# wengroup/matten

Measured on AMD Instinct MI355X. Metric: edge_tensor_products_per_sec, higher is better.
Workload: dtype f32; 1 GPU; configs[2]: synthetic fcc-64 crystals (64 atoms, cutoff 5 A, 1152 edges each), paper hparams lmax=4, eval forward backbone+out_layer, one batch per step per GPU; last conv layer run for its live outputs only (258/842 radial-weight columns: the irreps its only reader takes) -- `value` counts 4 edge-TP per edge all the same, `value_full_layers` is the rate with the full last layer; nodes_per_gpu=64000, edges_per_gpu=1152000, conv_layers=4

## Files before the change

### include/matten_hip.h

```cpp
#ifndef MATTEN_HIP_H
#define MATTEN_HIP_H

#include <stddef.h>
#include <stdint.h>

#ifdef __cplusplus
extern "C" {
#endif

typedef void* matten_stream_t;

#define MATTEN_OK 0
#define MATTEN_EINVAL (-1)
#define MATTEN_ELAUNCH (-2)
#define MATTEN_ENOMEM (-3)

int matten_abi_version(void);

#define MATTEN_RADIAL_MAX_MID 3

size_t matten_csr_workspace_bytes(int64_t n_edges, int64_t n_nodes);
int matten_csr_counting_max_avg_degree(void);
int matten_csr_build(const int64_t* edge_index, int64_t n_edges, int64_t n_nodes, int32_t* perm,
                     int32_t* rowptr, int32_t* src_sorted, void* workspace, size_t workspace_bytes,
                     int32_t* err_flag, matten_stream_t stream);

int64_t matten_csr_split_bound(int64_t n_nodes, int64_t n_edges, int64_t max_len);
int matten_csr_split(const int32_t* rowptr, int64_t n_nodes, int64_t n_edges, int64_t max_len, int32_t* vrowptr,
                     int64_t* vseg, const float* num_neigh, float* vnn, matten_stream_t stream);

size_t matten_group_workspace_bytes(int64_t n, int64_t n_keys);
int matten_group_by_key(const int64_t* key, int64_t n, int64_t n_keys, int32_t* order, int32_t* seg,
                        void* workspace, size_t workspace_bytes, int32_t* err_flag, matten_stream_t stream);

int matten_species_embed(const int64_t* atomic_numbers, int64_t n_nodes, const int64_t* z_to_index,
                         int64_t min_z, int64_t max_z, int64_t n_species, const float* weight ,
                         const float* bias , int64_t dim, int64_t* species_index, int32_t* species_i32,
                         float* node_feats, float* node_attrs, int32_t* err_flag, matten_stream_t stream);

int matten_edge_geom(const float* pos, const int64_t* edge_index, const float* edge_cell_shift,
                     const float* cell, int64_t n_cells, const int64_t* batch, const int32_t* perm,
                     int64_t n_edges, int64_t n_nodes, int lmax, int n_basis, float r_start, float r_end,
                     float* geom_sorted, float* sh_sorted, int sh_stride, float* edge_vectors, float* edge_lengths,
                     float* edge_attrs, float* edge_embedding, matten_stream_t stream);

int matten_radial_mlp(const float* geom_sorted, int64_t n_edges, int n_basis, float r_start, float r_end,
                      const float* w0p, int nb_pad, const float* w1p, const float* w2p, int hidden, int w_pad,
                      float act_cst, void* w_edge, int out_is_bf16, matten_stream_t stream);
int matten_radial_mlp_deep(const float* geom_sorted, int64_t n_edges, int n_basis, float r_start, float r_end,
                           const float* w0p, int nb_pad, const float* w_mid, int n_mid, const float* w2p, int hidden,
                           int w_pad, float act_cst, void* w_edge, int out_is_bf16, matten_stream_t stream);

int matten_tp_tile_nodes(void);
int matten_tp_paths(const float* x, int64_t d_in, const void* w_edge, int64_t w_pad, const float* sh_sorted,
                    int64_t sh_dim, const int32_t* rowptr, const int32_t* src_sorted, int64_t n_nodes,
                    const int32_t* path_entries, const int32_t* unit_start, int64_t n_entries,
                    int64_t units_per_tile, int64_t d_mid, float avg_num_neighbors, const float* num_neigh,
                    float* agg , int w_is_bf16, matten_stream_t stream);

int matten_agg_linear_max_mt(void);
int matten_agg_linear_block_chunks(void);
size_t matten_agg_linear_lds_bytes(int64_t w_stride, int64_t n_io, int64_t n_blocks);
size_t matten_agg_linear_max_lds_bytes(void);
int matten_agg_linear(const float* agg, int64_t ld, const int32_t* order, const int32_t* seg, int64_t n_species,
                      const float* wtab, int64_t w_stride, const int32_t* io_table, int64_t n_io,
                      const int32_t* blocks, int64_t n_blocks, const float* add, int64_t add_ld, int64_t d_out,
                      int64_t n_rows, float* out, matten_stream_t stream);
int matten_agg_linear_gate(const float* agg, int64_t ld, const int32_t* order, const int32_t* seg, int64_t n_species,
                           const float* wtab, int64_t w_stride, const int32_t* io_table, int64_t n_io,
                           const int32_t* blocks, int64_t n_blocks, const float* add, int64_t add_ld, int64_t d_out,
                           int64_t n_rows, const int32_t* cmeta, const float* act_cst, const float* bn_scale,
                           const float* bn_shift, int64_t d_act, float* out, matten_stream_t stream);
int matten_agg_linear_gate_sets(void);
int matten_radial_hidden(const float* geom_sorted, int64_t n_edges, int n_basis, float r_start, float r_end,
                         const float* w0p, int nb_pad, const float* w1p, int hidden, uint16_t* h2s,
                         const float* h_scale, matten_stream_t stream);
int matten_radial_hidden_multi(const float* geom_sorted, int64_t n_edges, int n_basis, float r_start, float r_end,
                               const float* const* w0p, int nb_pad, const float* const* w1p, int hidden,
                               uint16_t* const* h2s, const float* const* h_scale, int n_layers,
                               matten_stream_t stream);
int matten_radial_hidden_deep(const float* geom_sorted, int64_t n_edges, int n_basis, float r_start, float r_end,
                              const float* w0p, int nb_pad, const float* w_mid, int n_mid, int hidden, uint16_t* h2s,
                              const float* h_scale, matten_stream_t stream);
int matten_radial_hidden_multi_deep(const float* geom_sorted, int64_t n_edges, int n_basis, float r_start, float r_end,
                                    const float* const* w0p, int nb_pad, const float* const* w_mid, int n_mid, int hidden,
                                    uint16_t* const* h2s, const float* const* h_scale, int n_layers,
                                    matten_stream_t stream);
int matten_tp_fused(const float* x, int64_t d_in, const uint16_t* h2s, const float* w2p, int64_t w_pad,
                    const float* sh_sorted, int64_t sh_stride, const int32_t* rowptr, const int32_t* src_sorted,
                    int64_t n_nodes, const int32_t* group_entries, const int32_t* unit_map, int64_t n_entries,
                    int64_t units_per_tile, int64_t lds_floats_per_wave, int64_t d_mid, float avg_num_neighbors,
                    const float* num_neigh, const uint16_t* a_split, const float* a_scale_inv,
                    float* agg , matten_stream_t stream);

int matten_tp_max_cols(void);
int matten_tp_max_cols_l0(void);
int matten_tp_max_cols_l1(void);
int matten_tp_groups_hash(void);

int matten_species_linear(const float* x, int64_t d_in, const int32_t* order, const int32_t* seg, int64_t n_species,
                          const float* wp, int64_t w_stride, const int32_t* segs, int64_t n_segs, int64_t d_out,
                          const float* add, int64_t add_ld, int64_t n_rows, float* out, matten_stream_t stream);

int matten_species_linear_rows(const float* x, int64_t d_in, const int32_t* order, const int32_t* seg, int64_t n_species,
                               const float* wp, int64_t w_stride, const int32_t* segs, int64_t n_segs, int64_t d_out,
                               const float* add, int64_t add_ld, int64_t n_rows, float* out, matten_stream_t stream);

int matten_gate_bn(const float* x, int64_t d_in, const int32_t* meta, int64_t d_out, const float* act_cst,
                   const float* running_mean, const float* running_var, const float* bn_weight,
                   const float* bn_bias, float eps, int64_t n_rows, float* out, matten_stream_t stream);

int matten_segment_reduce(const float* x, int64_t dim, const int64_t* ptr, int64_t n_segments, int mean,
                          float* out, matten_stream_t stream);
int matten_segment_minmax(const float* x, int64_t dim, const int64_t* ptr, int64_t n_segments, int take_max, float* out,
                          int64_t* arg, matten_stream_t stream);
int matten_segment_minmax_bwd(const float* dy, int64_t dim, const int64_t* arg, int64_t n_segments, float* dx,
                              matten_stream_t stream);

int64_t matten_radial_mlp_bwd_small_slices(int64_t n_edges);
int64_t matten_radial_mlp_bwd_w2_ranges(int64_t n_edges, int64_t w_pad);
int matten_radial_mlp_bwd(const float* geom_sorted, int64_t n_edges, int n_basis, float r_start, float r_end,
                          const float* w0p, int nb_pad, const float* w1p, const float* w2p, int hidden, int w_pad,
                          int w_cols, const void* dw, int64_t dw_ld, int dw_is_bf16, float* h2_scratch,
                          float* part_small, float* part_w2, float scale0, float scale1, float scale2,
                          float* grad_small, float* grad_w2, matten_stream_t stream);
int64_t matten_radial_mlp_bwd_w2_ranges_deep(int64_t n_edges, int64_t w_pad, int n_mid);
int matten_radial_mlp_bwd_deep(const float* geom_sorted, int64_t n_edges, int n_basis, float r_start, float r_end,
                               const float* w0p, int nb_pad, const float* w_mid, int n_mid, const float* w2p, int hidden,
                               int w_pad, int w_cols, const void* dw, int64_t dw_ld, int dw_is_bf16, float* h2_scratch,
                               float* part_small, float* part_w2, float scale0, float scale1, float scale2,
                               float* grad_small, float* grad_w2, matten_stream_t stream);
int matten_radial_pack(const float* w0, const float* w1, const float* w2, int n_basis, int nb_pad, int w_cols, int w_pad,
                       float scale0, float scale1, float scale2, float* w0p, float* w1p, float* w2p,
                       matten_stream_t stream);
int matten_radial_pack_deep(const float* w0, const float* w_mid, int n_mid, const float* w2, int n_basis, int nb_pad,
                            int w_cols, int w_pad, float scale0, float scale1, float scale2, float* w0p, float* w_mid_p,
                            float* w2p, matten_stream_t stream);
int matten_radial_pack_cols(const float* w0, const float* w1, const float* w2, int n_basis, int nb_pad, int w_cols,
                            const int64_t* cols, int n_cols, int w_pad, float scale0, float scale1, float scale2, float* w0p,
                            float* w1p, float* w2p, matten_stream_t stream);
int matten_radial_h_scale(const float* w0, const float* w1, int n_basis, float r_start, float r_end, float act_cst,
                          float* out2, matten_stream_t stream);
int matten_radial_pack_cols_deep(const float* w0, const float* w_mid, int n_mid, const float* w2, int n_basis, int nb_pad,
                                 int w_cols, const int64_t* cols, int n_cols, int w_pad, float scale0, float scale1,
                                 float scale2, float* w0p, float* w_mid_p, float* w2p, matten_stream_t stream);
int matten_radial_h_scale_deep(const float* w0, const float* w_mid, int n_mid, int n_basis, float r_start, float r_end,
                               float act_cst, float* out2, matten_stream_t stream);
int matten_split_a_tiles(const float* w2p, int64_t w_pad, const int32_t* group_entries, int64_t n_entries,
                         const float* h_scale, uint16_t* frag, float* scale_inv, matten_stream_t stream);
int matten_gather_scale(const float* src, const int64_t* idx, const float* scale, int64_t n, int64_t scale_period,
                        int scale_by_source, float* out, const int64_t* perm2, float* out2, matten_stream_t stream);
int64_t matten_species_linear_wgrad_scratch_floats(int64_t n_rows, int64_t n_species, int64_t w_stride);

int matten_dense_rows(const float* x, int64_t n_in, const float* q, int64_t n_out, int64_t n_rows, float* out,
                      matten_stream_t stream);



int matten_tp_backward(const float* x, int64_t d_in, const void* w_edge, int64_t w_ld, const float* sh_sorted,
                       int64_t sh_stride, const int32_t* src_sorted, const int32_t* dst_sorted,
                       const int32_t* col_meta, int64_t n_cols, const uint8_t* nnz_ijk, const float* nnz_c,
                       const float* g_agg, int64_t d_mid, float avg_num_neighbors, const float* num_neigh,
                       int64_t n_edges, float* dx, void* dw, int64_t dw_ld, const int32_t* in_ptr,
                       const int32_t* in_cols, int64_t n_in, int edge_is_bf16 ,
                       matten_stream_t stream);

int matten_adam_step(float* params, const float* grads, float* exp_avg, float* exp_avg_sq, int64_t n, const float* step,
                     float lr, float beta1, float beta2, float eps, float weight_decay, matten_stream_t stream);

int matten_tp_backward_lit(const float* x, int64_t d_in, const void* w_edge, int64_t w_ld, const float* sh_sorted,
                           int64_t sh_stride, const int32_t* src_sorted, const int32_t* dst_sorted, const int32_t* blocks,
                           int64_t n_blocks, int64_t max_mul, const int32_t* paths, int64_t n_paths, const float* g_agg,
                           int64_t d_mid, float avg_num_neighbors, const float* num_neigh, int64_t n_edges, float* dx,
                           void* dw, int64_t dw_ld, int edge_is_bf16, int64_t n_nodes, const int32_t* out_ptr,
                           const int32_t* out_perm, float* dx_edges, int max_l, matten_stream_t stream);
int matten_tp_backward_lit_wfree(const float* x, int64_t d_in, const uint16_t* h2s, const uint16_t* frag, const float* w_inv,
                                 const float* sh_sorted, int64_t sh_stride, const int32_t* src_sorted,
                                 const int32_t* dst_sorted, const int32_t* blocks, int64_t n_blocks, int64_t sum_lanes,
                                 const int32_t* paths, int64_t n_paths, const float* g_agg, int64_t d_mid,
                                 float avg_num_neighbors, const float* num_neigh, int64_t n_edges, float* dx, void* dw,
                                 int64_t dw_ld, int edge_is_bf16, int64_t n_nodes, const int32_t* out_ptr,
                                 const int32_t* out_perm, float* dx_edges, int64_t lds_floats, int max_l, int max_mul,
                                 matten_stream_t stream);

int matten_species_linear_wgrad(const float* x, int64_t d_in, const float* dy, int64_t d_out, const int32_t* order,
                                const int32_t* seg, int64_t n_species, int64_t n_rows, const int32_t* segs,
                                int64_t n_segs, int64_t w_stride, float* dwp, float* scratch, matten_stream_t stream);

int matten_gate_bwd(const float* x, int64_t d_in, const int32_t* meta, int64_t d_out, const float* act_cst,
                    const float* dy, int64_t n_rows, float* dx, matten_stream_t stream);

int64_t matten_bn_scratch_floats(int64_t n_rows, int64_t dim);
int matten_bn_train_fwd(const float* x, int64_t dim, int64_t n_rows, const int32_t* col2chan, const int32_t* chan,
                        int64_t n_chan, const float* weight, const float* bias, float eps, float* mean, float* nu,
                        float* y, float* running_mean, float* running_var, float momentum, float* scratch,
                        matten_stream_t stream);
int matten_bn_train_bwd(const float* x, const float* dy, int64_t dim, int64_t n_rows, const int32_t* col2chan,
                        const int32_t* chan, int64_t n_chan, const float* mean, const float* nu, const float* weight,
                        float eps, float* A, float* B, float* dx, float* dweight, float* dbias, float* scratch,
                        matten_stream_t stream);

int matten_norm_act(const float* x, int64_t dim, int64_t n_rows, const int32_t* chan, int64_t n_chan, int act,
                    float epsilon, const float* running_mean, const float* running_var, const float* bn_weight,
                    const float* bn_bias, float bn_eps, float* y, matten_stream_t stream);
int matten_norm_act_bwd(const float* x, const float* dy, int64_t dim, int64_t n_rows, const int32_t* chan, int64_t n_chan,
                        int act, float epsilon, float* dx, matten_stream_t stream);

int matten_instance_norm_fwd(const float* x, int64_t dim, int64_t n_rows, const int64_t* seg_ptr, const int64_t* seg_of_row,
                             int64_t n_seg, const int32_t* col2chan, const int32_t* chan, int64_t n_chan,
                             const float* weight, const float* bias, float eps, float* mean, float* nu, float* y,
                             matten_stream_t stream);
int matten_instance_norm_bwd(const float* x, const float* dy, int64_t dim, int64_t n_rows, const int64_t* seg_ptr,
                             const int64_t* seg_of_row, int64_t n_seg, const int32_t* col2chan, const int32_t* chan,
                             int64_t n_chan, const float* mean, const float* nu, const float* weight, float eps, float* A,
                             float* B, float* dx, matten_stream_t stream);

int matten_segment_reduce_bwd(const float* dy, int64_t dim, const int64_t* ptr, int64_t n_segments, int mean, float* dx,
                              matten_stream_t stream);


int matten_graph_prep(const double* pos, const double* cell, const int64_t* ptr, int64_t n_crystals, double r_cut,
                      double* frac, double* bound, int64_t* batch, float* pos_f32, float* cell_f32,
                      matten_stream_t stream);
int matten_neighbor_count(const double* pos, const double* cell, const int64_t* ptr, const double* frac,
                          const double* bound, const int64_t* pair_ptr, double r_cut, int64_t n_crystals,
                          int64_t max_atoms, int32_t* counts, int32_t* counts_t, matten_stream_t stream);
int matten_neighbor_summary(const int64_t* offsets, const int64_t* pair_ptr, int64_t n_crystals, int64_t* out2,
                            matten_stream_t stream);
int matten_neighbor_fill(const double* pos, const double* cell, const int64_t* ptr, const double* frac,
                         const double* bound, const int64_t* pair_ptr, double r_cut, int64_t n_crystals,
                         int64_t max_atoms, const int64_t* offsets, int64_t n_edges, int64_t* edge_index,
                         float* edge_cell_shift, float* num_neigh, const int64_t* offsets_t, int64_t n_atoms,
                         int32_t* rowptr, int32_t* src_sorted, int32_t* perm, matten_stream_t stream);

#ifdef __cplusplus
}
#endif
#endif
```

### matten_amd/_lib.py

```python
from __future__ import annotations

import ctypes
import os
from ctypes import c_float, c_int, c_int32, c_int64, c_size_t, c_void_p

_HERE = os.path.dirname(os.path.abspath(__file__))
LIB_PATH = os.path.join(_HERE, "libmatten_hip.so")

ABI_VERSION = 45

P = c_void_p
SIGNATURES = {
    "matten_abi_version": (c_int, []),
    "matten_csr_workspace_bytes": (c_size_t, [c_int64, c_int64]),
    "matten_group_workspace_bytes": (c_size_t, [c_int64, c_int64]),
    "matten_csr_counting_max_avg_degree": (c_int, []),
    "matten_csr_build": (c_int, [P, c_int64, c_int64, P, P, P, P, c_size_t, P, P]),
    "matten_csr_split_bound": (c_int64, [c_int64, c_int64, c_int64]),
    "matten_csr_split": (c_int, [P, c_int64, c_int64, c_int64, P, P, P, P, P]),
    "matten_group_by_key": (c_int, [P, c_int64, c_int64, P, P, P, c_size_t, P, P]),
    "matten_species_embed": (c_int, [P, c_int64, P, c_int64, c_int64, c_int64, P, P, c_int64, P, P, P, P, P, P]),
    "matten_edge_geom": (c_int, [P, P, P, P, c_int64, P, P, c_int64, c_int64, c_int, c_int, c_float, c_float, P, P, c_int, P, P, P, P, P]),
    "matten_radial_mlp": (c_int, [P, c_int64, c_int, c_float, c_float, P, c_int, P, P, c_int, c_int, c_float, P, c_int, P]),
    "matten_radial_mlp_deep": (c_int, [P, c_int64, c_int, c_float, c_float, P, c_int, P, c_int, P, c_int, c_int, c_float, P, c_int,
                                       P]),
    "matten_tp_tile_nodes": (c_int, []),
    "matten_tp_paths": (c_int, [P, c_int64, P, c_int64, P, c_int64, P, P, c_int64, P, P, c_int64, c_int64, c_int64, c_float, P, P, c_int,
                                P]),
    "matten_radial_hidden_multi": (c_int, [P, c_int64, c_int, c_float, c_float, P, c_int, P, c_int, P, P, c_int, P]),
    "matten_radial_hidden_multi_deep": (c_int, [P, c_int64, c_int, c_float, c_float, P, c_int, P, c_int, c_int, P, P, c_int, P]),
    "matten_agg_linear_max_mt": (c_int, []),
    "matten_agg_linear_block_chunks": (c_int, []),
    "matten_agg_linear_lds_bytes": (c_size_t, [c_int64, c_int64, c_int64]),
    "matten_agg_linear_max_lds_bytes": (c_size_t, []),
    "matten_agg_linear": (c_int, [P, c_int64, P, P, c_int64, P, c_int64, P, c_int64, P, c_int64, P, c_int64, c_int64,
                                  c_int64, P, P]),
    "matten_agg_linear_gate": (c_int, [P, c_int64, P, P, c_int64, P, c_int64, P, c_int64, P, c_int64, P, c_int64, c_int64,
                                       c_int64, P, P, P, P, c_int64, P, P]),
    "matten_agg_linear_gate_sets": (c_int, []),
    "matten_radial_hidden": (c_int, [P, c_int64, c_int, c_float, c_float, P, c_int, P, c_int, P, P, P]),
    "matten_radial_hidden_deep": (c_int, [P, c_int64, c_int, c_float, c_float, P, c_int, P, c_int, c_int, P, P, P]),
    "matten_tp_max_cols": (c_int, []),
    "matten_tp_max_cols_l0": (c_int, []),
    "matten_tp_max_cols_l1": (c_int, []),
    "matten_tp_groups_hash": (c_int, []),
    "matten_tp_fused": (c_int, [P, c_int64, P, P, c_int64, P, c_int64, P, P, c_int64, P, P, c_int64, c_int64, c_int64, c_int64, c_float, P, P, P, P, P]),
    "matten_species_linear": (c_int, [P, c_int64, P, P, c_int64, P, c_int64, P, c_int64, c_int64, P, c_int64, c_int64, P, P]),
    "matten_species_linear_rows": (c_int, [P, c_int64, P, P, c_int64, P, c_int64, P, c_int64, c_int64, P, c_int64, c_int64, P, P]),
    "matten_radial_mlp_bwd_small_slices": (c_int64, [c_int64]),
    "matten_radial_mlp_bwd_w2_ranges": (c_int64, [c_int64, c_int64]),
    "matten_radial_mlp_bwd_w2_ranges_deep": (c_int64, [c_int64, c_int64, c_int]),
    "matten_radial_mlp_bwd": (c_int, [P, c_int64, c_int, c_float, c_float, P, c_int, P, P, c_int, c_int, c_int, P, c_int64,
                                      c_int, P, P, P, c_float, c_float, c_float, P, P, P]),
    "matten_radial_mlp_bwd_deep": (c_int, [P, c_int64, c_int, c_float, c_float, P, c_int, P, c_int, P, c_int, c_int, c_int, P,
                                           c_int64, c_int, P, P, P, c_float, c_float, c_float, P, P, P]),
    "matten_radial_pack": (c_int, [P, P, P, c_int, c_int, c_int, c_int, c_float, c_float, c_float, P, P, P, P]),
    "matten_radial_pack_deep": (c_int, [P, P, c_int, P, c_int, c_int, c_int, c_int, c_float, c_float, c_float, P, P, P, P]),
    "matten_radial_pack_cols": (c_int, [P, P, P, c_int, c_int, c_int, P, c_int, c_int, c_float, c_float, c_float, P, P, P, P]),
    "matten_radial_pack_cols_deep": (c_int, [P, P, c_int, P, c_int, c_int, c_int, P, c_int, c_int, c_float, c_float, c_float, P, P,
                                             P, P]),
    "matten_radial_h_scale": (c_int, [P, P, c_int, c_float, c_float, c_float, P, P]),
    "matten_radial_h_scale_deep": (c_int, [P, P, c_int, c_int, c_float, c_float, c_float, P, P]),
    "matten_split_a_tiles": (c_int, [P, c_int64, P, c_int64, P, P, P, P]),
    "matten_gather_scale": (c_int, [P, P, P, c_int64, c_int64, c_int, P, P, P, P]),
    "matten_species_linear_wgrad_scratch_floats": (c_int64, [c_int64, c_int64, c_int64]),
    "matten_tp_backward": (c_int, [P, c_int64, P, c_int64, P, c_int64, P, P, P, c_int64, P, P, P, c_int64, c_float, P, c_int64, P, P, c_int64,
                                   P, P, c_int64, c_int, P]),
    "matten_tp_backward_lit": (c_int, [P, c_int64, P, c_int64, P, c_int64, P, P, P, c_int64, c_int64, P, c_int64, P, c_int64, c_float,
                                       P, c_int64, P, P, c_int64, c_int, c_int64, P, P, P, c_int, P]),
    "matten_tp_backward_lit_wfree": (c_int, [P, c_int64, P, P, P, P, c_int64, P, P, P, c_int64, c_int64, P, c_int64, P, c_int64, c_float,
                                             P, c_int64, P, P, c_int64, c_int, c_int64, P, P, P, c_int64, c_int, c_int, P]),
    "matten_adam_step": (c_int, [P, P, P, P, c_int64, P, c_float, c_float, c_float, c_float, c_float, P]),
    "matten_species_linear_wgrad": (c_int, [P, c_int64, P, c_int64, P, P, c_int64, c_int64, P, c_int64, c_int64, P, P, P]),
    "matten_gate_bwd": (c_int, [P, c_int64, P, c_int64, P, P, c_int64, P, P]),
    "matten_bn_scratch_floats": (c_int64, [c_int64, c_int64]),
    "matten_bn_train_fwd": (c_int, [P, c_int64, c_int64, P, P, c_int64, P, P, c_float, P, P, P, P, P, c_float, P, P]),
    "matten_bn_train_bwd": (c_int, [P, P, c_int64, c_int64, P, P, c_int64, P, P, P, c_float, P, P, P, P, P, P, P]),
    "matten_norm_act": (c_int, [P, c_int64, c_int64, P, c_int64, c_int, c_float, P, P, P, P, c_float, P, P]),
    "matten_norm_act_bwd": (c_int, [P, P, c_int64, c_int64, P, c_int64, c_int, c_float, P, P]),
    "matten_instance_norm_fwd": (c_int, [P, c_int64, c_int64, P, P, c_int64, P, P, c_int64, P, P, c_float, P, P, P, P]),
    "matten_instance_norm_bwd": (c_int, [P, P, c_int64, c_int64, P, P, c_int64, P, P, c_int64, P, P, P, c_float, P, P, P, P]),
    "matten_segment_reduce_bwd": (c_int, [P, c_int64, P, c_int64, c_int, P, P]),
    "matten_graph_prep": (c_int, [P, P, P, c_int64, ctypes.c_double, P, P, P, P, P, P]),
    "matten_neighbor_count": (c_int, [P, P, P, P, P, P, ctypes.c_double, c_int64, c_int64, P, P, P]),
    "matten_neighbor_summary": (c_int, [P, P, c_int64, P, P]),
    "matten_neighbor_fill": (c_int, [P, P, P, P, P, P, ctypes.c_double, c_int64, c_int64, P, c_int64, P, P, P, P, c_int64,
                                     P, P, P, P]),
    "matten_gate_bn": (c_int, [P, c_int64, P, c_int64, P, P, P, P, P, c_float, c_int64, P, P]),
    "matten_segment_reduce": (c_int, [P, c_int64, P, c_int64, c_int, P, P]),
    "matten_segment_minmax": (c_int, [P, c_int64, P, c_int64, c_int, P, P, P]),
    "matten_segment_minmax_bwd": (c_int, [P, c_int64, P, c_int64, P, P]),
    "matten_dense_rows": (c_int, [P, c_int64, P, c_int64, c_int64, P, P]),
}

_lib = None


class MattenHipError(RuntimeError):
    pass


def load() -> ctypes.CDLL:
    global _lib
    if _lib is not None:
        return _lib
    if not os.path.exists(LIB_PATH):
        raise MattenHipError(
            f"{LIB_PATH} not found: the HIP extension is not built. matten_amd has no CPU fallback; "
            "run `make -C matten_amd/csrc` (needs hipcc, --offload-arch=gfx950)."
        )
    lib = ctypes.CDLL(LIB_PATH)
    for name, (res, args) in SIGNATURES.items():
        try:
            fn = getattr(lib, name)
        except AttributeError as e:
            raise MattenHipError(f"symbol {name} missing from {LIB_PATH}") from e
        fn.restype = res
        fn.argtypes = args
    v = lib.matten_abi_version()
    if v != ABI_VERSION:
        raise MattenHipError(f"ABI version mismatch: library {v}, python binding {ABI_VERSION}")
    _lib = lib
    return lib


_ERRORS = {-1: "MATTEN_EINVAL (bad argument)", -2: "MATTEN_ELAUNCH (HIP launch failed)", -3: "MATTEN_ENOMEM (workspace too small)"}


def check(rc: int, what: str) -> None:
    if rc != 0:
        raise MattenHipError(f"{what} failed: {_ERRORS.get(rc, rc)}")
```

### matten_amd/csrc/agg_linear.hip

```cpp
#include <atomic>

#include "common.h"

namespace {

typedef float f32x4 __attribute__((ext_vector_type(4)));

#ifndef AL_WAVES_PER_WG
#define AL_WAVES_PER_WG 8
#endif
constexpr int AL_WAVES = AL_WAVES_PER_WG;
constexpr int AL_ROWS = 16;
#ifndef AL_BLK_CHUNKS
#define AL_BLK_CHUNKS 4
#endif
#ifndef AL_MIN_BLOCKS
#define AL_MIN_BLOCKS 3
#endif
#ifndef AL_GATE_PREFETCH
#define AL_GATE_PREFETCH 1
#endif
constexpr int AL_BLK = AL_BLK_CHUNKS;
constexpr int AL_MAX_MT = 2;

constexpr int AL_STAGE_RS = 33;

struct AggIo {
    int chunk0, T, K, packed, a_off, out_off, mo, k0;
};
struct AggBlk {
    int chunk;
    int info;
    int t0;
    int pad;
};

struct Args {
    const float* agg;
    const int* order;
    const int* seg;
    const float* wtab;
    const AggIo* io;
    const AggBlk* blk;
    const float* add;
    float* out;
    int64_t ld;
    int n_species, w_stride, n_io, n_blk, add_ld, d_out, n_rows;
    const int4* cmeta;
    const float* act_cst;
    const float* bn_scale;
    const float* bn_shift;
    int out_ld;
};

__device__ __forceinline__ float al_act(int code, float v) {
    switch (code) {
        case 1: return v / (1.0f + expf(-v));
        case 2: return tanhf(v);
        case 3: return 1.0f / (1.0f + expf(-v));
        case 4: return (v > 20.0f ? v : log1pf(expf(v))) - 0.6931471805599453f;
        case 5: return fabsf(v);
        default: return v;
    }
}
constexpr int AL_GATE_SETS = 3;

#ifdef AL_WAVES_PER_EU
#define AL_OCC __attribute__((amdgpu_waves_per_eu(AL_WAVES_PER_EU, AL_WAVES_PER_EU)))
#else
#define AL_OCC
#endif
template <bool GATE>
__global__ __launch_bounds__(AL_WAVES * 64, AL_MIN_BLOCKS) AL_OCC void agg_linear_kernel(Args a) {
    extern __shared__ __attribute__((aligned(16))) float lds[];
    AggIo* io_l = reinterpret_cast<AggIo*>(lds + a.w_stride);
    AggBlk* blk_l = reinterpret_cast<AggBlk*>(io_l + a.n_io);
    float* stage_all = reinterpret_cast<float*>(blk_l + a.n_blk);
    int s = 0, blk = blockIdx.x, beg = 0, end = a.n_rows;
    if (a.order) {
        int* sseg = reinterpret_cast<int*>(stage_all);
        const int cap = AL_WAVES * (16 * AL_STAGE_RS + 16) - 4;
        if (a.n_species + 1 <= cap) {
            for (int i = threadIdx.x; i <= a.n_species; i += AL_WAVES * 64) sseg[i] = a.seg[i];
            __syncthreads();
            if (threadIdx.x == 0) {
                int b = blk, sp = 0;
                for (; sp < a.n_species; ++sp) {
                    const int nb = (sseg[sp + 1] - sseg[sp] + AL_WAVES * AL_ROWS - 1) / (AL_WAVES * AL_ROWS);
                    if (b < nb) break;
                    b -= nb;
                }
                sseg[cap] = sp;
                sseg[cap + 1] = b;
            }
            __syncthreads();
            s = sseg[cap];
            blk = sseg[cap + 1];
            if (s < a.n_species) beg = sseg[s], end = sseg[s + 1];
            __syncthreads();
        } else {
            for (; s < a.n_species; ++s) {
                beg = a.seg[s];
                end = a.seg[s + 1];
                const int nb = (end - beg + AL_WAVES * AL_ROWS - 1) / (AL_WAVES * AL_ROWS);
                if (blk < nb) break;
                blk -= nb;
            }
        }
    } else if (blk >= (a.n_rows + AL_WAVES * AL_ROWS - 1) / (AL_WAVES * AL_ROWS)) {
        s = a.n_species;
    }
    if (s >= a.n_species) return;
    {
        const f32x4* src = reinterpret_cast<const f32x4*>(a.wtab + (int64_t)s * a.w_stride);
        f32x4* dst = reinterpret_cast<f32x4*>(lds);
        for (int i = threadIdx.x; i < a.w_stride / 4; i += AL_WAVES * 64) dst[i] = src[i];
        const int* isrc = reinterpret_cast<const int*>(a.io);
        int* idst = reinterpret_cast<int*>(io_l);
        for (int i = threadIdx.x; i < a.n_io * 8; i += AL_WAVES * 64) idst[i] = isrc[i];
        const int* bsrc = reinterpret_cast<const int*>(a.blk);
        int* bdst = reinterpret_cast<int*>(blk_l);
        for (int i = threadIdx.x; i < a.n_blk * 4; i += AL_WAVES * 64) bdst[i] = bsrc[i];
    }
    __syncthreads();
    const int wave = __builtin_amdgcn_readfirstlane(threadIdx.x >> 6);
    const int lane = threadIdx.x & 63;
    const int g = lane >> 4, c = lane & 15;
    const int r0 = beg + (blk * AL_WAVES + wave) * AL_ROWS;
    if (r0 >= end) return;
    const int ri = min(r0 + c, end - 1);
    const bool row_ok = r0 + c < end;
    const int64_t row = a.order ? a.order[ri] : ri;
    const float* rp = a.agg + row * a.ld + 4 * g;
    const bool has_add = a.add != nullptr;
    float* stage = stage_all + wave * (16 * AL_STAGE_RS);
    int* rowid = reinterpret_cast<int*>(stage_all + AL_WAVES * 16 * AL_STAGE_RS) + wave * 16;
    if (g == 0) rowid[c] = row_ok ? (int)row : -1;
    const int fcol = lane & 31, frow = lane >> 5;

    int K = 0, d3 = 0, n_mt = 0, cw = 0, a_off = 0, out_off = 0, mo = 0, k0 = 0, kk = 1;
    auto load_io = [&](int ii) {
        const AggIo r = io_l[ii];
        K = __builtin_amdgcn_readfirstlane(r.K);
        d3 = __builtin_amdgcn_readfirstlane(r.packed & 255);
        n_mt = __builtin_amdgcn_readfirstlane((r.packed >> 8) & 255);
        cw = __builtin_amdgcn_readfirstlane((r.packed >> 16) & 255);
        a_off = __builtin_amdgcn_readfirstlane(r.a_off);
        out_off = __builtin_amdgcn_readfirstlane(r.out_off);
        mo = __builtin_amdgcn_readfirstlane(r.mo);
        k0 = __builtin_amdgcn_readfirstlane(r.k0);
        kk = __builtin_amdgcn_readfirstlane((r.packed >> 24) & 255);
    };
    f32x4 acc[AL_MAX_MT];
    float addv[8];
    auto zero_acc = [&]() {
#pragma unroll
        for (int mt = 0; mt < AL_MAX_MT; ++mt) acc[mt] = f32x4{0.f, 0.f, 0.f, 0.f};
    };
    int4 cm_row = {0, 0, 0, 0};
    float cst_row = 1.0f, bsc_row = 1.0f, bsh_row = 0.0f;
    int ocol = 0;
    auto open_row = [&]() {
        const int w = mo * kk;
        const int fc = min(fcol, w - 1), fv = fc / kk;
        ocol = out_off + fv * d3 + k0 + (fc - fv * kk);
#pragma unroll
        for (int p = 0; p < 8; ++p) {
            const int rid = max(rowid[2 * p + frow], 0);
            addv[p] = has_add ? a.add[(int64_t)rid * a.add_ld + ocol] : 0.0f;
        }
        if constexpr (GATE && AL_GATE_PREFETCH) {
            cm_row = a.cmeta[ocol];
            const int type = cm_row.x & 255, code = (cm_row.x >> 8) & 255;
            cst_row = code ? a.act_cst[code] : 1.0f;
            bsc_row = 1.0f, bsh_row = 0.0f;
            if (a.bn_scale && (type == 1 || type == 3)) bsc_row = a.bn_scale[cm_row.y], bsh_row = a.bn_shift[cm_row.y];
        }
    };
    auto close_unit = [&](int k) {
#pragma unroll
        for (int mt = 0; mt < AL_MAX_MT; ++mt) {
            if (mt < n_mt) {
#pragma unroll
                for (int i = 0; i < 4; ++i) {
                    const int v = 16 * mt + 4 * g + i;
                    if (v < mo) stage[c * AL_STAGE_RS + v * kk + (k - k0)] = acc[mt][i];
                }
            }
        }
    };
    float gate_reg[GATE ? AL_GATE_SETS : 1][8];
    auto flush_row = [&]() {
        const int w = mo * kk;
        __builtin_amdgcn_s_waitcnt(0xc07f);
        __builtin_amdgcn_wave_barrier();
        if constexpr (GATE) {
            const int4 cm = AL_GATE_PREFETCH ? cm_row : a.cmeta[ocol];
            const int type = cm.x & 255, code = (cm.x >> 8) & 255;
            float cst = cst_row, bsc = bsc_row, bsh = bsh_row;
            if (!AL_GATE_PREFETCH) {
                cst = code ? a.act_cst[code] : 1.0f;
                if (a.bn_scale && (type == 1 || type == 3)) bsc = a.bn_scale[cm.y], bsh = a.bn_shift[cm.y];
            }
            const int src_lane = (cm.z & 31) | (frow << 5);
#pragma unroll
            for (int p = 0; p < 8; ++p) {
                const int r = 2 * p + frow;
                const int rid = rowid[r];
                float v = stage[r * AL_STAGE_RS + min(fcol, w - 1)] + addv[p];
                float gv = __shfl(gate_reg[0][p], src_lane);
#pragma unroll
                for (int st = 1; st < AL_GATE_SETS; ++st) {
                    const float o = __shfl(gate_reg[st][p], src_lane);
                    gv = cm.w == st ? o : gv;
                }
                if (type == 2) {
                    const float act = (code ? al_act(code, v) : v) * cst;
#pragma unroll
                    for (int st = 0; st < AL_GATE_SETS; ++st)
                        if (cm.w == st && fcol < w) gate_reg[st][p] = act;
                } else if (fcol < w && rid >= 0 && type != 0) {
                    if (type == 1) v = (code ? al_act(code, v) : v) * cst;
                    else v = v * gv;
                    a.out[(int64_t)rid * a.out_ld + cm.y] = fmaf(v, bsc, bsh);
                }
            }
            __builtin_amdgcn_wave_barrier();
            return;
        }
#pragma unroll
        for (int p = 0; p < 8; ++p) {
            const int r = 2 * p + frow;
            const int rid = rowid[r];
#ifdef AL_ABL_NO_STORE
            if (fcol < w && rid >= 0 && addv[p] == 12345.678f)
#elif defined(AL_ABL_SMALL_OUT)
            if (fcol < w && rid >= 0) a.out[(int64_t)(rid & 63) * a.d_out + ocol] = stage[r * AL_STAGE_RS + fcol] + addv[p];
            if (false)
#else
            if (fcol < w && rid >= 0)
#endif
                a.out[(int64_t)rid * a.d_out + ocol] = stage[r * AL_STAGE_RS + fcol] + addv[p];
        }
        __builtin_amdgcn_wave_barrier();
    };
    auto fetch = [&](int j, f32x4* __restrict__ buf) {
        const AggBlk d = blk_l[j];
        const int c0 = __builtin_amdgcn_readfirstlane(d.chunk);
        const int n = __builtin_amdgcn_readfirstlane(d.info & 255);
#pragma unroll
        for (int i = 0; i < AL_BLK; ++i) {
#ifdef AL_NT_LOADS
            buf[i] = __builtin_nontemporal_load(reinterpret_cast<const f32x4*>(rp + 16 * (c0 + min(i, n - 1))));
#else
            buf[i] = *reinterpret_cast<const f32x4*>(rp + 16 * (c0 + min(i, n - 1)));
#endif
        }
    };
    auto step = [&](int j, const f32x4* __restrict__ cur, f32x4* __restrict__ nxt) {
        fetch(min(j + 1, a.n_blk - 1), nxt);
        const AggBlk d = blk_l[j];
        const int info = __builtin_amdgcn_readfirstlane(d.info);
        const int n = info & 255, k = (info >> 12) & 255;
        const int t0 = __builtin_amdgcn_readfirstlane(d.t0);
        const int cc = min(c, cw - 1);
#pragma unroll
        for (int i = 0; i < AL_BLK; ++i) {
            if (i < n) {
                f32x4 b = cur[i];
#ifdef AL_ABL_NO_LDS
                const f32x4 afix = {1.f, 2.f, 3.f, (float)i};
#endif
                const int t = t0 + i;
                const int slot0 = 16 * t + 4 * g;
#pragma unroll
                for (int sst = 0; sst < 4; ++sst) b[sst] = slot0 + sst < K ? b[sst] : 0.0f;
                const float* ab = lds + a_off + ((t * n_mt * 4 + g) * cw + cc) * 4;
#pragma unroll
                for (int mt = 0; mt < AL_MAX_MT; ++mt) {
                    if (mt < n_mt) {
#ifdef AL_ABL_NO_LDS
                        f32x4 a4 = afix;
#else
                        f32x4 a4 = *reinterpret_cast<const f32x4*>(ab + mt * 4 * cw * 4);
#endif
                        if (c >= cw) a4 = f32x4{0.f, 0.f, 0.f, 0.f};
#ifdef AL_ABL_NO_MFMA
                        acc[mt][0] += a4[0] * b[0] + a4[1] * b[1] + a4[2] * b[2] + a4[3] * b[3];
#else
#pragma unroll
                        for (int sst = 0; sst < 4; ++sst)
                            acc[mt] = __builtin_amdgcn_mfma_f32_16x16x4f32(a4[sst], b[sst], acc[mt], 0, 0, 0);
#endif
                    }
                }
            }
        }
        if ((info >> 9) & 1) {
            close_unit(k);
            zero_acc();
            if ((info >> 10) & 1) {
                flush_row();
                if (j + 1 < a.n_blk) {
                    load_io((__builtin_amdgcn_readfirstlane(blk_l[j + 1].info) >> 20) & 4095);
                    open_row();
                }
            }
        }
    };
#pragma unroll
    for (int st = 0; st < (GATE ? AL_GATE_SETS : 1); ++st)
#pragma unroll
        for (int p = 0; p < 8; ++p) gate_reg[st][p] = 0.0f;
    f32x4 bufa[AL_BLK], bufb[AL_BLK];
    __builtin_amdgcn_s_waitcnt(0xc07f);
    __builtin_amdgcn_wave_barrier();
    load_io(0);
    zero_acc();
    open_row();
    fetch(0, bufa);
    for (int j = 0; j < a.n_blk; j += 2) {
        step(j, bufa, bufb);
        if (j + 1 < a.n_blk) step(j + 1, bufb, bufa);
    }
}

}

constexpr size_t AL_MAX_LDS = 80 * 1024;
extern "C" size_t matten_agg_linear_lds_bytes(int64_t w_stride, int64_t n_io, int64_t n_blocks) {
    return sizeof(float) * (size_t)w_stride + sizeof(AggIo) * (size_t)n_io + sizeof(AggBlk) * (size_t)n_blocks +
           sizeof(float) * AL_WAVES * (16 * AL_STAGE_RS + 16);
}
extern "C" size_t matten_agg_linear_max_lds_bytes(void) { return AL_MAX_LDS; }
extern "C" int matten_agg_linear_max_mt(void) { return AL_MAX_MT; }
extern "C" int matten_agg_linear_block_chunks(void) { return AL_BLK; }

static int agg_linear_launch(const float* agg, int64_t ld, const int32_t* order, const int32_t* seg, int64_t n_species,
                             const float* wtab, int64_t w_stride, const int32_t* io_table, int64_t n_io,
                             const int32_t* blocks, int64_t n_blocks, const float* add, int64_t add_ld, int64_t d_out,
                             int64_t n_rows, float* out, const int32_t* cmeta, const float* act_cst, const float* bn_scale,
                             const float* bn_shift, int64_t out_ld, hipStream_t stream) {
    if (n_rows < 0 || ld <= 0 || (ld & 3) || n_species <= 0 || w_stride <= 0 || (w_stride & 3) || n_io <= 0 ||
        n_blocks <= 0 || d_out <= 0 || out_ld <= 0)
        return MATTEN_EINVAL;
    if (n_rows == 0) return MATTEN_OK;
    if (!agg || !wtab || !io_table || !blocks || !out) return MATTEN_EINVAL;
    if ((order == nullptr) != (seg == nullptr)) return MATTEN_EINVAL;
    if (!order && n_species != 1) return MATTEN_EINVAL;
    if (add && add_ld < d_out) return MATTEN_EINVAL;
    if (cmeta && !act_cst) return MATTEN_EINVAL;
    if ((bn_scale == nullptr) != (bn_shift == nullptr)) return MATTEN_EINVAL;
    const size_t lds = matten_agg_linear_lds_bytes(w_stride, n_io, n_blocks);
    if (lds > AL_MAX_LDS) return MATTEN_EINVAL;
    if (lds > 64 * 1024) {
        static std::atomic<uint64_t> raised{0};
        int dev = 0;
        if (hipGetDevice(&dev) != hipSuccess || dev < 0) return MATTEN_ELAUNCH;
        const uint64_t bit = dev < 64 ? (uint64_t)1 << dev : 0;
        if (!bit || !(raised.load(std::memory_order_acquire) & bit)) {
            if (hipFuncSetAttribute((const void*)agg_linear_kernel<false>, hipFuncAttributeMaxDynamicSharedMemorySize,
                                    (int)AL_MAX_LDS) != hipSuccess ||
                hipFuncSetAttribute((const void*)agg_linear_kernel<true>, hipFuncAttributeMaxDynamicSharedMemorySize,
                                    (int)AL_MAX_LDS) != hipSuccess)
                return MATTEN_ELAUNCH;
            raised.fetch_or(bit, std::memory_order_release);
        }
    }
    const int64_t grid = matten_cdiv(n_rows, AL_WAVES * AL_ROWS) + n_species;
    if (grid >= ((int64_t)1 << 31) || n_rows >= ((int64_t)1 << 31)) return MATTEN_EINVAL;
    Args a{agg, order, seg, wtab, (const AggIo*)io_table, (const AggBlk*)blocks, add, out, ld, (int)n_species,
           (int)w_stride, (int)n_io, (int)n_blocks, (int)add_ld, (int)d_out, (int)n_rows, (const int4*)cmeta, act_cst,
           bn_scale, bn_shift, (int)out_ld};
    if (cmeta) agg_linear_kernel<true><<<(unsigned)grid, AL_WAVES * 64, lds, stream>>>(a);
    else agg_linear_kernel<false><<<(unsigned)grid, AL_WAVES * 64, lds, stream>>>(a);
    MATTEN_LAUNCH_CHECK();
    return MATTEN_OK;
}

extern "C" int matten_agg_linear(const float* agg, int64_t ld, const int32_t* order, const int32_t* seg,
                                 int64_t n_species, const float* wtab, int64_t w_stride, const int32_t* io_table,
                                 int64_t n_io, const int32_t* blocks, int64_t n_blocks, const float* add,
                                 int64_t add_ld, int64_t d_out, int64_t n_rows, float* out, matten_stream_t stream_) {
    return agg_linear_launch(agg, ld, order, seg, n_species, wtab, w_stride, io_table, n_io, blocks, n_blocks, add, add_ld,
                             d_out, n_rows, out, nullptr, nullptr, nullptr, nullptr, d_out, (hipStream_t)stream_);
}

extern "C" int matten_agg_linear_gate_sets(void) { return AL_GATE_SETS; }

extern "C" int matten_agg_linear_gate(const float* agg, int64_t ld, const int32_t* order, const int32_t* seg,
                                      int64_t n_species, const float* wtab, int64_t w_stride, const int32_t* io_table,
                                      int64_t n_io, const int32_t* blocks, int64_t n_blocks, const float* add,
                                      int64_t add_ld, int64_t d_out, int64_t n_rows, const int32_t* cmeta,
                                      const float* act_cst, const float* bn_scale, const float* bn_shift, int64_t d_act,
                                      float* out, matten_stream_t stream_) {
    if (!cmeta || d_act <= 0) return MATTEN_EINVAL;
    return agg_linear_launch(agg, ld, order, seg, n_species, wtab, w_stride, io_table, n_io, blocks, n_blocks, add, add_ld,
                             d_out, n_rows, out, cmeta, act_cst, bn_scale, bn_shift, d_act, (hipStream_t)stream_);
}
```

### matten_amd/csrc/edge.hip

```cpp
#include "common.h"
#include "sh.h"

namespace {

constexpr int SH_TILE_RS = 36;

template <int LMAX>
__global__ __launch_bounds__(256) void edge_geom_kernel(const float* __restrict__ pos, const int64_t* __restrict__ edge_index,
                                 const float* __restrict__ shift, const float* __restrict__ cell, int64_t n_cells,
                                 const int64_t* __restrict__ batch, const int32_t* __restrict__ perm, int64_t E,
                                 int64_t N, int n_basis, float r_start, float r_end, float4* __restrict__ geom_sorted,
                                 float* __restrict__ sh_sorted, int sh_stride, float* __restrict__ edge_vectors,
                                 float* __restrict__ edge_lengths, float* __restrict__ edge_attrs,
                                 float* __restrict__ edge_embedding) {
    constexpr int SH = (LMAX + 1) * (LMAX + 1);
    __shared__ __attribute__((aligned(16))) float sh_tile[4 * 64 * SH_TILE_RS];
    const int64_t e_raw = (int64_t)blockIdx.x * blockDim.x + threadIdx.x;
    if (e_raw - (threadIdx.x & 63) >= E) return;
    const bool live = e_raw < E;
    const int64_t e = live ? e_raw : E - 1;
    int64_t o = perm ? (int64_t)perm[e] : e;
    int64_t i = edge_index[o];
    int64_t j = edge_index[E + o];
    i = i < 0 ? 0 : (i >= N ? N - 1 : i);
    j = j < 0 ? 0 : (j >= N ? N - 1 : j);
    float vx = pos[3 * j + 0] - pos[3 * i + 0];
    float vy = pos[3 * j + 1] - pos[3 * i + 1];
    float vz = pos[3 * j + 2] - pos[3 * i + 2];
    if (cell) {
        int64_t b = (n_cells > 1 && batch) ? batch[i] : 0;
        b = b < 0 ? 0 : (b >= n_cells ? n_cells - 1 : b);
        const float* c = cell + 9 * b;
        float s0 = shift[3 * o + 0], s1 = shift[3 * o + 1], s2 = shift[3 * o + 2];
        vx += s0 * c[0] + s1 * c[3] + s2 * c[6];
        vy += s0 * c[1] + s1 * c[4] + s2 * c[7];
        vz += s0 * c[2] + s1 * c[5] + s2 * c[8];
    }
    float len = sqrtf(vx * vx + vy * vy + vz * vz);
    if (live) geom_sorted[e] = make_float4(vx, vy, vz, len);

    float y[SH];
    matten::real_sh<LMAX>(vx, vy, vz, len, y);
    if (sh_stride == 32) {
        float* tile = sh_tile + (threadIdx.x >> 6) * (64 * SH_TILE_RS);
        const int lane = threadIdx.x & 63;
#pragma unroll
        for (int q = 0; q < 8; ++q)
            *reinterpret_cast<float4*>(tile + lane * SH_TILE_RS + 4 * q) =
                make_float4(4 * q < SH ? y[4 * q < SH ? 4 * q : 0] : 0.0f,
                            4 * q + 1 < SH ? y[4 * q + 1 < SH ? 4 * q + 1 : 0] : 0.0f,
                            4 * q + 2 < SH ? y[4 * q + 2 < SH ? 4 * q + 2 : 0] : 0.0f,
                            4 * q + 3 < SH ? y[4 * q + 3 < SH ? 4 * q + 3 : 0] : 0.0f);
        __builtin_amdgcn_s_waitcnt(0xc07f);
        __builtin_amdgcn_wave_barrier();
        const int64_t e0 = e_raw - lane;
        const int64_t n_here = E - e0 < 64 ? E - e0 : 64;
        float4* dst = reinterpret_cast<float4*>(sh_sorted + e0 * 32);
#pragma unroll
        for (int i = 0; i < 8; ++i) {
            const int f = i * 64 + lane;
            if ((f >> 3) < n_here)
                dst[f] = *reinterpret_cast<const float4*>(tile + (f >> 3) * SH_TILE_RS + 4 * (f & 7));
        }
    } else if (live) {
#pragma unroll
        for (int k = 0; k < SH; ++k) sh_sorted[e * sh_stride + k] = y[k];
        for (int k = SH; k < sh_stride; ++k) sh_sorted[e * sh_stride + k] = 0.0f;
    }
    if (!live) return;

    if (edge_vectors) {
        edge_vectors[3 * o + 0] = vx;
        edge_vectors[3 * o + 1] = vy;
        edge_vectors[3 * o + 2] = vz;
    }
    if (edge_lengths) edge_lengths[o] = len;
    if (edge_attrs) {
#pragma unroll
        for (int k = 0; k < SH; ++k) edge_attrs[o * SH + k] = y[k];
    }
    if (edge_embedding) {
        for (int k = 0; k < n_basis; ++k)
            edge_embedding[o * n_basis + k] = matten::bessel_basis(len, k, n_basis, r_start, r_end);
    }
}

__global__ void species_embed_kernel(const int64_t* __restrict__ Z, int64_t N, const int64_t* __restrict__ lut,
                                     int64_t min_z, int64_t max_z, int64_t S, const float* __restrict__ W,
                                     const float* __restrict__ b, int64_t dim, int64_t* __restrict__ species_index,
                                     int32_t* __restrict__ species_i32, float* __restrict__ feats,
                                     float* __restrict__ attrs, int32_t* err_flag) {
    int64_t n = (int64_t)blockIdx.x * blockDim.y + threadIdx.y;
    if (n >= N) return;
    int64_t z = Z[n];
    int64_t idx = -1;
    if (z < min_z || z > max_z) {
        if (threadIdx.x == 0) atomicOr(err_flag, 2);
    } else {
        idx = lut[z - min_z];
        if (idx < 0 || idx >= S) {
            if (threadIdx.x == 0) atomicOr(err_flag, 4);
            idx = -1;
        }
    }
    if (threadIdx.x == 0) {
        if (species_index) species_index[n] = idx;
        if (species_i32) species_i32[n] = (int32_t)(idx < 0 ? 0 : idx);
    }
    int64_t s = idx < 0 ? 0 : idx;
    for (int64_t d = threadIdx.x; d < dim; d += blockDim.x) feats[n * dim + d] = W[d * S + s] + b[d];
    if (attrs)
        for (int64_t c = threadIdx.x; c < S; c += blockDim.x) attrs[n * S + c] = (c == idx) ? 1.0f : 0.0f;
}

}

extern "C" int matten_species_embed(const int64_t* atomic_numbers, int64_t n_nodes, const int64_t* z_to_index,
                                    int64_t min_z, int64_t max_z, int64_t n_species, const float* weight,
                                    const float* bias, int64_t dim, int64_t* species_index, int32_t* species_i32,
                                    float* node_feats, float* node_attrs, int32_t* err_flag,
                                    matten_stream_t stream_) {
    hipStream_t stream = (hipStream_t)stream_;
    if (n_nodes < 0 || dim <= 0 || n_species <= 0) return MATTEN_EINVAL;
    if (n_nodes == 0) return MATTEN_OK;
    if (!atomic_numbers || !z_to_index || !weight || !bias || !node_feats || !err_flag) return MATTEN_EINVAL;
    dim3 block(16, 16);
    species_embed_kernel<<<(unsigned)matten_cdiv(n_nodes, 16), block, 0, stream>>>(
        atomic_numbers, n_nodes, z_to_index, min_z, max_z, n_species, weight, bias, dim, species_index, species_i32,
        node_feats, node_attrs, err_flag);
    MATTEN_LAUNCH_CHECK();
    return MATTEN_OK;
}

extern "C" int matten_edge_geom(const float* pos, const int64_t* edge_index, const float* edge_cell_shift,
                                const float* cell, int64_t n_cells, const int64_t* batch, const int32_t* perm,
                                int64_t n_edges, int64_t n_nodes, int lmax, int n_basis, float r_start, float r_end,
                                float* geom_sorted, float* sh_sorted, int sh_stride, float* edge_vectors, float* edge_lengths,
                                float* edge_attrs, float* edge_embedding, matten_stream_t stream_) {
    hipStream_t stream = (hipStream_t)stream_;
    if (n_edges < 0 || n_nodes < 0 || (n_edges > 0 && n_nodes == 0) || lmax < 0 || lmax > 4 || n_basis < 0 || sh_stride < (lmax + 1) * (lmax + 1)) return MATTEN_EINVAL;
    if (n_edges == 0) return MATTEN_OK;
    if (!pos || !edge_index || !geom_sorted || !sh_sorted) return MATTEN_EINVAL;
    if (cell && !edge_cell_shift) return MATTEN_EINVAL;
    const int T = 256;
    unsigned grid = (unsigned)matten_cdiv(n_edges, T);
#define LAUNCH(L)                                                                                              \
    edge_geom_kernel<L><<<grid, T, 0, stream>>>(pos, edge_index, edge_cell_shift, cell, n_cells, batch, perm,  \
                                                n_edges, n_nodes, n_basis, r_start, r_end, (float4*)geom_sorted, \
                                                sh_sorted, sh_stride, edge_vectors, edge_lengths, edge_attrs, edge_embedding)
    switch (lmax) {
        case 0: LAUNCH(0); break;
        case 1: LAUNCH(1); break;
        case 2: LAUNCH(2); break;
        case 3: LAUNCH(3); break;
        default: LAUNCH(4); break;
    }
#undef LAUNCH
    MATTEN_LAUNCH_CHECK();
    return MATTEN_OK;
}
```

### matten_amd/csrc/node.hip

```cpp
#include "common.h"

namespace {

__device__ __forceinline__ float apply_act(int code, float v) {
    switch (code) {
        case 1: return v / (1.0f + expf(-v));
        case 2: return tanhf(v);
        case 3: return 1.0f / (1.0f + expf(-v));
        case 4: return (v > 20.0f ? v : log1pf(expf(v))) - 0.6931471805599453f;
        case 5: return fabsf(v);
        default: return v;
    }
}

#ifndef GB_R
#define GB_R 16
#endif
#ifndef GB_U
#define GB_U 8
#endif
constexpr int GB_ROWS = GB_R, GB_UNROLL = GB_U;
__global__ __launch_bounds__(256) void gate_bn_kernel(const float* __restrict__ x, int d_in,
                                                           const int4* __restrict__ meta, int d_out,
                                                           const float* __restrict__ act_cst,
                                                           const float* __restrict__ running_mean,
                                                           const float* __restrict__ running_var,
                                                           const float* __restrict__ bn_weight,
                                                           const float* __restrict__ bn_bias, float eps, int64_t n_rows,
                                                           float* __restrict__ out) {
    const int o = blockIdx.y * blockDim.x + threadIdx.x;
    if (o >= d_out) return;
    const int4 m = meta[o];
    const int act = m.z & 0xff, gact = (m.z >> 8) & 0xff;
    const float ca = act ? act_cst[act] : 1.0f, cg = gact ? act_cst[gact] : 1.0f;
    float scale = 1.0f, shift = 0.0f;
    if (bn_weight) {
        const int bn_idx = m.w & 0xffff, mean_idx = (m.w >> 16) & 0xffff;
        scale = bn_weight[bn_idx] / sqrtf(running_var[bn_idx] + eps);
        if (mean_idx != 0xffff) shift = bn_bias[mean_idx] - running_mean[mean_idx] * scale;
    }
    const int gcol = m.y < 0 ? m.x : m.y;
    const int64_t row0 = (int64_t)blockIdx.x * GB_ROWS;
    const int rows = (int)min((int64_t)GB_ROWS, n_rows - row0);
    for (int r0 = 0; r0 < rows; r0 += GB_UNROLL) {
        float a[GB_UNROLL], b[GB_UNROLL];
#pragma unroll
        for (int i = 0; i < GB_UNROLL; ++i) {
            const int64_t r = row0 + min(r0 + i, rows - 1);
            a[i] = x[r * d_in + m.x];
            b[i] = x[r * d_in + gcol];
        }
#pragma unroll
        for (int i = 0; i < GB_UNROLL; ++i) {
            if (r0 + i < rows) {
                float v = a[i];
                if (m.y < 0) {
                    if (act) v = apply_act(act, v) * ca;
                } else {
                    float gte = b[i];
                    if (gact) gte = apply_act(gact, gte) * cg;
                    v = v * gte;
                }
                out[(row0 + r0 + i) * d_out + o] = bn_weight ? fmaf(v, scale, shift) : v;
            }
        }
    }
}


__global__ void segment_reduce_kernel(const float* __restrict__ x, int dim, const int64_t* __restrict__ ptr,
                                      int64_t n_seg, int mean, float* __restrict__ out) {
    int64_t idx = (int64_t)blockIdx.x * blockDim.x + threadIdx.x;
    if (idx >= n_seg * dim) return;
    int64_t b = idx / dim;
    int c = (int)(idx - b * dim);
    int64_t beg = ptr[b], end = ptr[b + 1];
    float s = 0.0f;
    int64_t n = beg;
    for (; n + 8 <= end; n += 8) {
        float v[8];
#pragma unroll
        for (int i = 0; i < 8; ++i) v[i] = x[(n + i) * dim + c];
#pragma unroll
        for (int i = 0; i < 8; ++i) s += v[i];
    }
    for (; n < end; ++n) s += x[n * dim + c];
    if (mean) {
        float cnt = (float)(end - beg);
        s = s / (cnt < 1.0f ? 1.0f : cnt);
    }
    out[idx] = s;
}

__global__ void segment_minmax_kernel(const float* __restrict__ x, int dim, const int64_t* __restrict__ ptr, int64_t n_seg,
                                      int take_max, float* __restrict__ out, int64_t* __restrict__ arg) {
    int64_t idx = (int64_t)blockIdx.x * blockDim.x + threadIdx.x;
    if (idx >= n_seg * dim) return;
    const int64_t b = idx / dim;
    const int c = (int)(idx - b * dim);
    const int64_t beg = ptr[b], end = ptr[b + 1];
    float best = 0.0f;
    int64_t at = -1;
    for (int64_t n = beg; n < end; ++n) {
        const float v = x[n * dim + c];
        if (at < 0 || (take_max ? v > best : v < best)) best = v, at = n;
    }
    out[idx] = best;
    if (arg) arg[idx] = at;
}

__global__ void segment_minmax_bwd_kernel(const float* __restrict__ dy, int dim, const int64_t* __restrict__ arg,
                                          int64_t n_seg, float* __restrict__ dx) {
    int64_t idx = (int64_t)blockIdx.x * blockDim.x + threadIdx.x;
    if (idx >= n_seg * dim) return;
    const int64_t at = arg[idx];
    if (at >= 0) dx[at * dim + (idx % dim)] = dy[idx];
}

__global__ void dense_rows_kernel(const float* __restrict__ x, int n_in, const float* __restrict__ q, int n_out,
                                  int64_t n_rows, float* __restrict__ out) {
    int64_t idx = (int64_t)blockIdx.x * blockDim.x + threadIdx.x;
    if (idx >= n_rows * n_out) return;
    int64_t b = idx / n_out;
    int c = (int)(idx - b * n_out);
    float s = 0.0f;
    for (int k = 0; k < n_in; ++k) s += x[b * n_in + k] * q[k * n_out + c];
    out[idx] = s;
}

}

extern "C" int matten_gate_bn(const float* x, int64_t d_in, const int32_t* meta, int64_t d_out, const float* act_cst,
                              const float* running_mean, const float* running_var, const float* bn_weight,
                              const float* bn_bias, float eps, int64_t n_rows, float* out, matten_stream_t stream_) {
    hipStream_t stream = (hipStream_t)stream_;
    if (n_rows < 0 || d_in <= 0 || d_out <= 0) return MATTEN_EINVAL;
    if (n_rows == 0) return MATTEN_OK;
    if (!x || !meta || !act_cst || !out) return MATTEN_EINVAL;
    if (bn_weight && (!running_var || !running_mean || !bn_bias)) return MATTEN_EINVAL;
    const int TC = (int)(d_out >= 256 ? 256 : 64 * matten_cdiv(d_out, 64));
    dim3 grid((unsigned)matten_cdiv(n_rows, GB_ROWS), (unsigned)matten_cdiv(d_out, TC));
    gate_bn_kernel<<<grid, TC, 0, stream>>>(x, (int)d_in, (const int4*)meta, (int)d_out, act_cst, running_mean, running_var,
                                            bn_weight, bn_bias, eps, n_rows, out);
    MATTEN_LAUNCH_CHECK();
    return MATTEN_OK;
}

extern "C" int matten_segment_reduce(const float* x, int64_t dim, const int64_t* ptr, int64_t n_segments, int mean,
                                     float* out, matten_stream_t stream_) {
    hipStream_t stream = (hipStream_t)stream_;
    if (n_segments < 0 || dim <= 0) return MATTEN_EINVAL;
    if (n_segments == 0) return MATTEN_OK;
    if (!x || !ptr || !out) return MATTEN_EINVAL;
    const int T = 256;
    segment_reduce_kernel<<<(unsigned)matten_cdiv(n_segments * dim, T), T, 0, stream>>>(x, (int)dim, ptr, n_segments,
                                                                                        mean, out);
    MATTEN_LAUNCH_CHECK();
    return MATTEN_OK;
}

extern "C" int matten_segment_minmax(const float* x, int64_t dim, const int64_t* ptr, int64_t n_segments, int take_max,
                                     float* out, int64_t* arg, matten_stream_t stream_) {
    hipStream_t stream = (hipStream_t)stream_;
    if (n_segments < 0 || dim <= 0) return MATTEN_EINVAL;
    if (n_segments == 0) return MATTEN_OK;
    if (!x || !ptr || !out) return MATTEN_EINVAL;
    const int T = 256;
    segment_minmax_kernel<<<(unsigned)matten_cdiv(n_segments * dim, T), T, 0, stream>>>(x, (int)dim, ptr, n_segments,
                                                                                        take_max, out, arg);
    MATTEN_LAUNCH_CHECK();
    return MATTEN_OK;
}

extern "C" int matten_segment_minmax_bwd(const float* dy, int64_t dim, const int64_t* arg, int64_t n_segments, float* dx,
                                         matten_stream_t stream_) {
    hipStream_t stream = (hipStream_t)stream_;
    if (n_segments < 0 || dim <= 0) return MATTEN_EINVAL;
    if (n_segments == 0) return MATTEN_OK;
    if (!dy || !arg || !dx) return MATTEN_EINVAL;
    const int T = 256;
    segment_minmax_bwd_kernel<<<(unsigned)matten_cdiv(n_segments * dim, T), T, 0, stream>>>(dy, (int)dim, arg, n_segments, dx);
    MATTEN_LAUNCH_CHECK();
    return MATTEN_OK;
}

extern "C" int matten_dense_rows(const float* x, int64_t n_in, const float* q, int64_t n_out, int64_t n_rows,
                                 float* out, matten_stream_t stream_) {
    hipStream_t stream = (hipStream_t)stream_;
    if (n_rows < 0 || n_in <= 0 || n_out <= 0) return MATTEN_EINVAL;
    if (n_rows == 0) return MATTEN_OK;
    if (!x || !q || !out) return MATTEN_EINVAL;
    const int T = 256;
    dense_rows_kernel<<<(unsigned)matten_cdiv(n_rows * n_out, T), T, 0, stream>>>(x, (int)n_in, q, (int)n_out, n_rows,
                                                                                  out);
    MATTEN_LAUNCH_CHECK();
    return MATTEN_OK;
}

extern "C" int matten_abi_version(void) { return 45; }
```

### matten_amd/model_factory/tfn_scalar_tensor.py

```python
from collections import OrderedDict
from typing import Any, Dict, Optional, Tuple

import torch
from torch import Tensor

from ..model.model import BaseModel
from ..nn._nequip import SphericalHarmonicEdgeAttrs
from ..nn.conv import PointConv, PointConvWithActivation
from ..nn.embedding import EdgeLengthEmbedding, SpeciesEmbedding
from ..nn.nodewise import NodewiseLinear, NodewiseReduce
from ..nn.utils import SpeciesLinear
from ..o3 import Irreps
from ..utils import CartesianTensor, ToCartesian
from .utils import create_sequential_module, validate_hparams

OUT_FIELD_NAME = "my_model_output"


def create_model(hparams: Dict[str, Any], dataset_hparams: Dict[str, Any], pooling: bool = True):
    validate_hparams(hparams, dataset_hparams)
    use_atom_feats = hparams.get("use_atom_feats", False)
    atom_feats_dim = dataset_hparams.get("atom_feats_size", None)
    materialize = bool(hparams.get("materialize_intermediates", False))

    layers = OrderedDict()
    layers["one_hot"] = (
        SpeciesEmbedding,
        {
            "embedding_dim": hparams["species_embedding_dim"],
            "allowed_species": dataset_hparams["allowed_species"],
            "use_atom_feats": use_atom_feats,
            "atom_feats_dim": atom_feats_dim,
            "materialize": materialize,
        },
    )
    layers["spharm_edges"] = (
        SphericalHarmonicEdgeAttrs,
        {"irreps_edge_sh": hparams["irreps_edge_sh"], "materialize": materialize},
    )
    layers["radial_basis"] = (
        EdgeLengthEmbedding,
        {
            "num_basis": hparams["num_radial_basis"],
            "start": hparams["radial_basis_start"],
            "end": hparams["radial_basis_end"],
            "basis": hparams["radial_basis_type"],
            "materialize": materialize,
        },
    )

    num_neigh = hparams["average_num_neighbors"]
    if isinstance(num_neigh, str) and num_neigh.lower() == "auto":
        num_neigh = dataset_hparams["average_num_neighbors"]

    conv_kwargs = {
        "conv_layer_irreps": hparams["conv_layer_irreps"],
        "fc_num_hidden_layers": hparams["invariant_layers"],
        "fc_hidden_size": hparams["invariant_neurons"],
        "avg_num_neighbors": num_neigh,
    }
    for i in range(hparams["num_layers"]):
        layers[f"layer{i}_convnet"] = (
            PointConvWithActivation,
            dict(conv_kwargs, activation_type=hparams["nonlinearity_type"], normalization=hparams["normalization"]),
        )
    layers["conv_layer_last"] = (PointConv, dict(conv_kwargs))
    layers["conv_to_output_hidden"] = (
        NodewiseLinear,
        {"irreps_out": hparams["conv_to_output_hidden_irreps_out"], "out_field": OUT_FIELD_NAME},
    )
    if pooling:
        layers["output_pooling"] = (
            NodewiseReduce,
            {"field": OUT_FIELD_NAME, "out_field": OUT_FIELD_NAME, "reduce": hparams["reduce"]},
        )
    backbone = create_sequential_module(modules=layers)
    link_radial_mlps(backbone)
    eliminate_dead_outputs(backbone)
    return backbone


def eliminate_dead_outputs(backbone) -> None:
    from ..data.irreps import DataKey

    mods = list(backbone._modules.values())
    for i in range(len(mods) - 1):
        conv, head = mods[i], mods[i + 1]
        if type(conv) is not PointConv or not isinstance(head, NodewiseLinear):
            continue
        if head.field != DataKey.NODE_FEATURES or head.out_field == DataKey.NODE_FEATURES:
            continue
        if any(getattr(m, "field", None) == DataKey.NODE_FEATURES or isinstance(m, (PointConv, PointConvWithActivation))
               for m in mods[i + 2:]):
            continue
        read = {ir for _, ir in Irreps(head.irreps_out[head.out_field])}
        kept = Irreps([(m, ir) for m, ir in conv.irreps_out[DataKey.NODE_FEATURES] if ir in read])
        if kept.dim == 0 or kept.dim == conv.irreps_out[DataKey.NODE_FEATURES].dim:
            continue
        if head.build_kept_input(kept) and not conv.build_inference_view(kept):
            head.__dict__["_kept"] = None


def link_radial_mlps(backbone) -> None:
    from ..nn.utils import RadialMLP, link_radial_group

    groups = {}
    for m in backbone.modules():
        if isinstance(m, RadialMLP):
            groups.setdefault(tuple(m.hs[:3]), []).append(m)
    for group in groups.values():
        for i in range(0, len(group), 8):
            if len(group[i:i + 8]) > 1:
                link_radial_group(group[i:i + 8])


class ScalarTensorModel(BaseModel):
    def __init__(
        self,
        tasks=None,
        backbone_hparams: Dict[str, Any] = None,
        dataset_hparams: Dict[str, Any] = None,
        optimizer_hparams: Dict[str, Any] = None,
        lr_scheduler_hparams: Dict[str, Any] = None,
        trainer_hparams: Dict[str, Any] = None,
        data_hparams: Dict[str, Any] = None,
        **kwargs,
    ):
        super().__init__()
        hparams = {
            "tasks": tasks,
            "backbone_hparams": backbone_hparams,
            "dataset_hparams": dataset_hparams,
            "optimizer_hparams": optimizer_hparams,
            "lr_scheduler_hparams": lr_scheduler_hparams,
            "trainer_hparams": trainer_hparams,
            "data_hparams": data_hparams,
        }
        self.optimizer_hparams = optimizer_hparams
        self.lr_scheduler_hparams = lr_scheduler_hparams
        self.backbone, extra = self.init_backbone(backbone_hparams, dataset_hparams)
        self.extra_layers_dict = torch.nn.ModuleDict(extra)
        self.tasks = self.init_tasks(tasks)
        self._init_training_shell(hparams)

    def init_backbone(self, backbone_hparams, dataset_hparams=None) -> Tuple[torch.nn.Module, Dict]:
        backbone = create_model(backbone_hparams, dataset_hparams)
        formula = backbone_hparams["output_formula"].lower()
        irreps_out = Irreps("0e") if formula == "scalar" else CartesianTensor(formula=formula)
        irreps_in = backbone_hparams["conv_to_output_hidden_irreps_out"]
        extra = {"out_layer": SpeciesLinear(irreps_in, None, irreps_out)}
        if backbone_hparams["output_format"] == "cartesian" and formula != "scalar":
            self.to_cartesian = ToCartesian(formula)
        else:
            self.to_cartesian = None
        return backbone, extra

    @staticmethod
    def init_tasks(tasks) -> Dict[str, Any]:
        from .task import TensorRegressionTask

        if tasks is None:
            tasks = "elastic_tensor_full"
        if isinstance(tasks, str):
            return {tasks: TensorRegressionTask(name=tasks)}
        if isinstance(tasks, dict):
            return {k: (t if t is not None else TensorRegressionTask(name=k)) for k, t in tasks.items()}
        if isinstance(tasks, (list, tuple)):
            return {getattr(t, "name", t): (TensorRegressionTask(name=t) if isinstance(t, str) else t) for t in tasks}
        return {tasks.name: tasks}

    def set_input_checks(self, mode) -> None:
        for m in self.modules():
            if hasattr(m, "check_species"):
                if hasattr(m, "finish_checks"):
                    m.finish_checks()
                m.check_species = mode

    def finish_input_checks(self) -> None:
        for m in self.modules():
            if hasattr(m, "finish_checks"):
                m.finish_checks()

    def preprocess_batch(self, batch):
        if hasattr(batch, "to") and not isinstance(batch, dict):
            batch = batch.to(self.device)
        if hasattr(batch, "tensor_property_to_dict"):
            y = getattr(batch, "y", None) or {}
            labels = {name: y[name] for name in self.tasks if name in y}
            graphs = batch.tensor_property_to_dict()
        else:
            dev = self.device
            graphs = {k: (v.to(dev) if isinstance(v, Tensor) and v.device != dev else v) for k, v in batch.items()}
            labels = {name: graphs[name] for name in self.tasks if name in graphs}
        return graphs, labels

    def decode(self, model_input) -> Dict[str, Tensor]:
        out = self.backbone(model_input)[OUT_FIELD_NAME]
        out = self.extra_layers_dict["out_layer"](out)
        if self.to_cartesian is not None:
            out = self.to_cartesian(out)
        names = list(self.tasks.keys())
        assert len(names) == 1, f"only works for 1 target, get{len(names)}"
        return {names[0]: out}

    def transform_prediction(self, preds, task_name: str = "elastic_tensor_full"):
        task = self.tasks.get(task_name)
        normalizer = getattr(task, "normalizer", None)
        if normalizer is None:
            return {task_name: preds[task_name]}
        if hasattr(normalizer, "normalizers"):
            return {task_name: normalizer.inverse(preds[task_name], task_name)}
        return {task_name: normalizer.inverse(preds[task_name])}

    def transform_target(self, target, task_name: str = "elastic_tensor_full"):
        if task_name not in target:
            return target
        return self.transform_prediction(target, task_name)

    def forward(self, batch, mode: Optional[str] = None, task_name: str = "elastic_tensor_full", **kwargs):
        graphs, labels = self.preprocess_batch(batch)
        if mode is None or mode.lower() == "none":
            preds = self.decode(graphs, **kwargs)
            preds = self.transform_prediction(preds, task_name=task_name)
            labels = self.transform_target(labels, task_name=task_name)
        elif mode == "backbone":
            preds = self.backbone(graphs, **kwargs)
        else:
            raise ValueError(f"Expect mode to be one of {(None, 'backbone')}; got {mode}")
        return preds, labels
```

### matten_amd/nn/conv.py

```python
from typing import Dict

import torch

import numpy as np

from .. import autograd as _ag
from .. import ops
from ..data.irreps import DataKey, ModuleIrreps
from ..o3 import Irreps
from ._tables import DerivedWeight, DeviceTables, WeightSlice
from .utils import ActivationLayer, NormalizationLayer, SpeciesLinear, UVUTensorProduct


import os as _os

GATE_APPLIED = "_amd_gate_applied"
GATE_FUSE = _os.environ.get("MATTEN_GATE_FUSE", "1") != "0"
KEPT_ONLY = "_amd_kept_irreps_only"
DEAD_PATH_ELIMINATION = _os.environ.get("MATTEN_DEAD_PATH_ELIMINATION", "1") != "0"
AGG_KM_MIN_ROWS = int(_os.environ.get("MATTEN_AGG_KM_MIN_ROWS", "8192"))


class PointConv(ModuleIrreps, torch.nn.Module):
    def __init__(
        self,
        irreps_in: Dict[str, Irreps],
        conv_layer_irreps: Irreps,
        fc_num_hidden_layers: int = 1,
        fc_hidden_size: int = 8,
        avg_num_neighbors: int = None,
    ):
        super().__init__()
        self.avg_num_neighbors = avg_num_neighbors
        self.init_irreps(irreps_in)
        self.__dict__["_ctor"] = dict(irreps_in=dict(irreps_in), fc_num_hidden_layers=fc_num_hidden_layers,
                                      fc_hidden_size=fc_hidden_size, avg_num_neighbors=avg_num_neighbors)
        self.__dict__["_view"] = None
        feats_in = self.irreps_in[DataKey.NODE_FEATURES]
        n_species = self.irreps_in[DataKey.NODE_ATTRS].dim
        edge_attrs = self.irreps_in[DataKey.EDGE_ATTRS]
        conv_layer_irreps = Irreps(conv_layer_irreps)

        self.lin1 = SpeciesLinear(feats_in, n_species, feats_in)
        self.tp = UVUTensorProduct(
            feats_in,
            edge_attrs,
            conv_layer_irreps,
            mlp_input_size=self.irreps_in[DataKey.EDGE_EMBEDDING].dim,
            mlp_hidden_size=fc_hidden_size,
            mlp_num_hidden_layers=fc_num_hidden_layers,
            mlp_activation="silu",
        )
        self.lin2 = SpeciesLinear(self.tp.irreps_out, n_species, conv_layer_irreps)
        self.sc = SpeciesLinear(feats_in, n_species, conv_layer_irreps)
        self.irreps_out[DataKey.NODE_FEATURES] = conv_layer_irreps
        self._lin1_sc = None
        self._lin1_sc_packed = DerivedWeight(self._pack_lin1_sc)
        from .. import plan as _plan
        import os
        self.agg_plan = None
        if self.tp.impl == "fused" and os.environ.get("MATTEN_AGG_LAYOUT", "km") == "km":
            ap = _plan.plan_agg_linear(self.tp.plan, n_species, conv_layer_irreps)
            if ap is not None and self._agg_fits(ap):
                self.agg_plan = ap
                self._agg_tables = DeviceTables(entries=ap.entries, io=ap.io_table, blocks=ap.blocks, gather=ap.gather,
                                                scale=ap.scale)
                self._agg_wtab = DerivedWeight(self._pack_agg_weights)

    def _pack_lin1_sc(self, w1: torch.Tensor, w2: torch.Tensor) -> torch.Tensor:
        return torch.cat([self.lin1._pack(w1), self.sc._pack(w2)], dim=1).contiguous()

    def _fused_lin1_sc_tables(self):
        if self._lin1_sc is None:
            p1, p2 = self.lin1.plan, self.sc.plan
            if len(p1.passes) != 1 or len(p2.passes) != 1 or not (p1.fully_covered and p2.fully_covered):
                self._lin1_sc = False
            else:
                seg2 = p2.passes[0].copy()
                seg2[:, 3] += p1.w_stride
                seg2[:, 5] += p1.d_out
                segs = np.concatenate([p1.passes[0], seg2])
                segs = segs[np.argsort(segs[:, 0], kind="stable")]
                self._lin1_sc = DeviceTables(meta=segs)
        return self._lin1_sc

    @staticmethod
    def _agg_fits(ap) -> bool:
        from .. import _lib
        try:
            lib = _lib.load()
        except Exception:
            return 4 * ap.w_stride <= 40 * 1024
        return lib.matten_agg_linear_lds_bytes(ap.w_stride, len(ap.io_table), len(ap.blocks)) <= lib.matten_agg_linear_max_lds_bytes()

    def _pack_agg_weights(self, w: torch.Tensor) -> torch.Tensor:
        t, dev = self._agg_tables, w.device
        gather, scale = t.get("gather", dev), t.get("scale", dev)
        return torch.where(gather >= 0, w[gather.clamp(min=0)] * scale[None, :], w.new_zeros(())).contiguous()

    def build_inference_view(self, kept_irreps) -> bool:
        kept = Irreps(kept_irreps).simplify()
        full_out = self.sc.irreps_out
        if any(sum(1 for _, ir2 in irr if ir2 == ir) != 1 for irr in (full_out, self.lin2.irreps_in) for _, ir in irr):
            return False
        if any(sum(1 for m2, ir2 in full_out if ir2 == ir and m2 == m) != 1 for m, ir in kept) or kept.dim >= full_out.dim:
            return False
        try:
            v = PointConv(conv_layer_irreps=kept, **self._ctor)
        except Exception:
            return False

        from .. import plan as _plan

        m_sc, m_l2 = _plan.linear_flat_submap(v.sc.plan, self.sc.plan), _plan.linear_flat_submap(v.lin2.plan, self.lin2.plan)
        fullp = {(q.i_in1, q.i_sh, q.l3, q.p3): q for q in self.tp.plan.paths}
        cols = []
        for q in v.tp.plan.paths:
            f = fullp.get((q.i_in1, q.i_sh, q.l3, q.p3))
            if f is None or f.mul != q.mul:
                return False
            cols.append(np.arange(f.w_off, f.w_off + f.mul))
        if m_sc is None or m_l2 is None or not cols:
            return False
        v.lin1 = self.lin1
        mlp, full = v.tp.weight_nn, self.tp.weight_nn
        last = len(full.hs) - 2
        for i in range(last):
            setattr(mlp, f"layer{i}", getattr(full, f"layer{i}"))
        mlp.__dict__["_hidden_from"] = full
        for mod in (v.sc, v.lin2, getattr(mlp, f"layer{last}")):
            del mod._parameters["weight"]
        v.__dict__["_slices"] = (WeightSlice(m_sc), WeightSlice(m_l2), WeightSlice(np.concatenate(cols), dim=1))
        self.__dict__["_view"] = v
        return True

    def _view_forward(self, data, differentiable: bool):
        v = self._view
        s_sc, s_l2, s_w2 = v._slices
        pick = (lambda sl, w: sl.select(w)) if differentiable else (lambda sl, w: sl.get(w))
        last = f"layer{len(self.tp.weight_nn.hs) - 2}"
        targets = ((v.sc, s_sc, self.sc.weight), (v.lin2, s_l2, self.lin2.weight),
                   (getattr(v.tp.weight_nn, last), s_w2, getattr(self.tp.weight_nn, last).weight))
        for mod, sl, w in targets:
            mod.__dict__["weight"] = pick(sl, w)
        try:
            return v(data)
        finally:
            if differentiable:
                for mod, _, _ in targets:
                    mod.__dict__["weight"] = None

    def forward(self, data: DataKey.Type) -> DataKey.Type:
        if self._view is not None and DEAD_PATH_ELIMINATION:
            data = self._view_forward(data, _ag.needs_grad_lazy(lambda: (data[DataKey.NODE_FEATURES], *_ag.params_of(self))))
            data[KEPT_ONLY] = True
            return data
        data.pop(KEPT_ONLY, None)
        x = data[DataKey.NODE_FEATURES]
        species = data[DataKey.AMD_SPECIES]
        fused = None if _ag.needs_grad(x, self.lin1.weight, self.sc.weight) else self._fused_lin1_sc_tables()
        if fused:
            wp = self._lin1_sc_packed.get(self.lin1.weight, self.sc.weight)
            d1, d2 = self.lin1.plan.d_out, self.sc.plan.d_out
            both = ops.species_linear(x, species, wp, self.lin1.plan.w_stride + self.sc.plan.w_stride,
                                      [fused.get("meta", x.device)], d1 + d2)
            x1, self_connection = both[:, :d1], both[:, d1:]
        else:
            self_connection = self.sc(x, species)
            x1 = self.lin1(x, species)
        if (self.agg_plan is not None and x1.shape[0] >= AGG_KM_MIN_ROWS
                and not _ag.needs_grad_lazy(lambda: (x1, self_connection, self.lin2.weight, *_ag.params_of(self.tp.weight_nn)))):
            ap, t, dev = self.agg_plan, self._agg_tables, x1.device
            agg = self.tp(x1, data, self.avg_num_neighbors, out_layout=(t.get("entries", dev), ap.ld))
            gate = self.__dict__.get("_gate_fuse")
            if gate is not None:
                cmeta, act_cst, d_act, bn_scale, bn_shift = gate
                data[DataKey.NODE_FEATURES] = ops.agg_linear_gate(
                    agg, species, self._agg_wtab.get(self.lin2.weight), t.get("io", dev), t.get("blocks", dev), ap.d_out,
                    cmeta, act_cst, d_act, add=self_connection, bn_scale=bn_scale, bn_shift=bn_shift)
                data[GATE_APPLIED] = True
                return data
            data[DataKey.NODE_FEATURES] = ops.agg_linear(agg, species, self._agg_wtab.get(self.lin2.weight),
                                                         t.get("io", dev), t.get("blocks", dev), ap.d_out,
                                                         add=self_connection)
            return data
        agg = self.tp(x1, data, self.avg_num_neighbors)
        data[DataKey.NODE_FEATURES] = self.lin2(agg, species, add=self_connection)
        return data


class PointConvWithActivation(ModuleIrreps, torch.nn.Module):
    def __init__(
        self,
        irreps_in: Dict[str, Irreps],
        conv_layer_irreps: Irreps,
        fc_num_hidden_layers: int = 1,
        fc_hidden_size: int = 8,
        avg_num_neighbors: int = None,
        activation_type: str = "gate",
        activation_scalars: Dict[str, str] = {"e": "silu", "o": "tanh"},
        activation_gates: Dict[str, str] = {"e": "sigmoid", "o": "tanh"},
        normalization: str = None,
    ):
        super().__init__()
        self.init_irreps(irreps_in)
        self.act = ActivationLayer(
            self.irreps_in[DataKey.NODE_FEATURES],
            self.irreps_in[DataKey.EDGE_ATTRS],
            Irreps(conv_layer_irreps),
            activation_type=activation_type,
            activation_scalars=activation_scalars,
            activation_gates=activation_gates,
        )
        self.conv = PointConv(
            irreps_in=self.irreps_in,
            conv_layer_irreps=self.act.irreps_in,
            fc_num_hidden_layers=fc_num_hidden_layers,
            fc_hidden_size=fc_hidden_size,
            avg_num_neighbors=avg_num_neighbors,
        )
        self.norm = NormalizationLayer(self.act.irreps_out, method=normalization)
        self.irreps_out[DataKey.NODE_FEATURES] = self.act.irreps_out

    def _gate_fuse_args(self, dev):
        if not GATE_FUSE or self.conv.agg_plan is None or getattr(self.act, "activation_type", "gate") != "gate":
            return None
        if self.norm.method not in ("batch", "none", None):
            return None
        bn = self.norm.n
        if bn is not None and bn.training:
            return None
        fuse = self.__dict__.get("_fuse_tables")
        if fuse is None:
            from .. import plan as _plan

            cm = _plan.plan_agg_gate(self.conv.agg_plan, self.act.plan)
            fuse = False if cm is None else DeviceTables(cmeta=cm)
            self.__dict__["_fuse_tables"] = fuse
            self.__dict__["_fuse_bn"] = DerivedWeight(self._fold_bn)
        if fuse is False:
            return None
        scale = shift = None
        if bn is not None:
            scale, shift = self._fuse_bn.get(bn.running_mean, bn.running_var, bn.weight, bn.bias)
        return (fuse.get("cmeta", dev), self.act._tables.get("act_cst", dev), self.act.plan.irreps_out.dim, scale, shift)

    def _fold_bn(self, rm, rv, w, b):
        meta = torch.as_tensor(np.asarray(self.act.plan.meta).reshape(-1, 4)[:, 3].astype(np.int64), device=w.device)
        bn_idx, mean_idx = meta & 0xFFFF, (meta >> 16) & 0xFFFF
        scale = (w / torch.sqrt(rv + self.norm.n.eps))[bn_idx]
        has_mean = mean_idx != 0xFFFF
        mi = torch.where(has_mean, mean_idx, torch.zeros_like(mean_idx))
        shift = torch.where(has_mean, b[mi] - rm[mi] * scale, torch.zeros_like(scale))
        return scale.contiguous(), shift.contiguous()

    def forward(self, data: DataKey.Type) -> DataKey.Type:
        x = data[DataKey.NODE_FEATURES]
        fuse = None
        if not _ag.needs_grad_lazy(lambda: (x, *_ag.params_of(self.conv))) and x.shape[0] >= AGG_KM_MIN_ROWS:
            fuse = self._gate_fuse_args(x.device)
        self.conv.__dict__["_gate_fuse"] = fuse
        try:
            data = self.conv(data)
        finally:
            self.conv.__dict__["_gate_fuse"] = None
        if data.pop(GATE_APPLIED, False):
            return data
        data[DataKey.NODE_FEATURES] = self.act(data[DataKey.NODE_FEATURES], self.norm, data)
        return data
```

### matten_amd/nn/embedding.py

```python
from typing import Dict, List, Tuple

import numpy as np
import torch

from .. import ops
from ..data.irreps import DataKey, ModuleIrreps
from ..o3 import Irreps


class _AtomicNumberToIndex(torch.nn.Module):

    def __init__(self, allowed_atomic_numbers: List[int]):
        super().__init__()
        allowed = torch.as_tensor(sorted(allowed_atomic_numbers), dtype=torch.long)
        lut = torch.full((int(allowed.max() - allowed.min()) + 1,), -1, dtype=torch.long)
        lut[allowed - allowed.min()] = torch.arange(len(allowed), dtype=torch.long)
        self.register_buffer("_min_Z", allowed.min())
        self.register_buffer("_max_Z", allowed.max())
        self.register_buffer("_num_species", torch.as_tensor(len(allowed)))
        self.register_buffer("_Z_to_index", lut)
        self._host = (int(allowed.min()), int(allowed.max()), len(allowed))
        self._allowed = [int(z) for z in allowed]

    @property
    def num_species(self):
        return self._num_species

    def raise_for_flags(self, flags: int, atomic_numbers: torch.Tensor):
        if flags & 2:
            raise RuntimeError(
                "Invalid atomic numbers. Expect atomic numbers to be in the range "
                f"[{self._host[0]}, {self._host[1]}], but got min {int(atomic_numbers.min())} "
                f"and max {int(atomic_numbers.max())}"
            )
        if flags & 4:
            z = atomic_numbers.cpu()
            for i, n in enumerate(z.tolist()):
                if n not in self._allowed:
                    raise RuntimeError(
                        f"Expect atomic numbers to be in {self._allowed}, "
                        f"got invalid atomic numbers `{n}` for data point `{i}`."
                    )

    def forward(self, atomic_numbers: torch.Tensor) -> torch.Tensor:
        lo, hi, _ = self._host
        if atomic_numbers.min() < lo or atomic_numbers.max() > hi:
            self.raise_for_flags(2, atomic_numbers)
        index = self._Z_to_index[atomic_numbers - lo]
        if index.min() < 0:
            self.raise_for_flags(4, atomic_numbers)
        return index


class SpeciesEmbedding(ModuleIrreps, torch.nn.Module):
    def __init__(
        self,
        irreps_in: Dict[str, Irreps] = None,
        embedding_dim: int = 16,
        num_species: int = None,
        allowed_species: List[int] = None,
        out_fields: Tuple[str] = (DataKey.NODE_ATTRS, DataKey.NODE_FEATURES),
        use_atom_feats: bool = False,
        atom_feats_dim: int = None,
        materialize: bool = False,
        check_species: bool = True,
    ):
        super().__init__()
        if allowed_species is not None and num_species is not None:
            raise ValueError("allowed_species and num_species cannot both be provided.")
        if allowed_species is None:
            raise NotImplementedError("matten_amd needs `allowed_species` (every shipped config provides it)")
        if use_atom_feats and atom_feats_dim is None:
            raise ValueError("`atom_feats_dim` must be provided if `use_atom_feats` is True.")
        self.use_atom_feats = use_atom_feats
        self.embedding_dim = embedding_dim
        self.out_fields = out_fields
        self.materialize = materialize
        self.check_species = check_species
        self.atomic_number_to_index = _AtomicNumberToIndex(allowed_species)
        self.num_species = len(allowed_species)
        self.init_irreps(
            irreps_in,
            {DataKey.NODE_ATTRS: Irreps(f"{self.num_species}x0e"),
             DataKey.NODE_FEATURES: Irreps(f"{embedding_dim + (atom_feats_dim if use_atom_feats else 0)}x0e")},
        )
        self.linear = torch.nn.Linear(self.num_species, embedding_dim)

    def finish_checks(self) -> None:
        pending, self._pending = getattr(self, "_pending", None), None
        if pending is None:
            return
        ev, host, Z, n_nodes = pending
        ev.synchronize()
        self._raise_for(host.tolist(), Z, n_nodes)

    def _raise_for(self, flags, Z, n_nodes) -> None:
        if flags[0]:
            self.atomic_number_to_index.raise_for_flags(flags[0], Z)
        if flags[1] & 1:
            rng = f"[0, {n_nodes})" if n_nodes is not None else "the batch's node range"
            raise IndexError(f"edge_index holds node ids outside {rng} (a malformed batch)")

    def raise_for_last_flags(self, n_nodes=None) -> None:
        flags_dev = getattr(self, "_last_flags", None)
        if flags_dev is None:
            return
        self._raise_for(flags_dev.tolist(), self._last_Z, n_nodes)

    def forward(self, data: DataKey.Type) -> DataKey.Type:
        a2i = self.atomic_number_to_index
        lo, hi, S = a2i._host
        if DataKey.SPECIES_INDEX in data:
            Z = data[DataKey.SPECIES_INDEX]
            lut = torch.arange(S, dtype=torch.int64, device=Z.device)
            lo, hi = 0, S - 1
            provided = True
        elif DataKey.ATOMIC_NUMBERS in data:
            Z, lut, provided = data[DataKey.ATOMIC_NUMBERS], a2i._Z_to_index, False
        else:
            raise ValueError("Nothing in `data` to encode. Need either species_index or atomic_numbers")
        flags_dev = torch.zeros(3, dtype=torch.int32, device=Z.device)
        sidx, s32, feats, attrs, _ = ops.species_embed(
            Z, lut, lo, hi, S, self.linear.weight, self.linear.bias, want_attrs=self.materialize, err=flags_dev[0:1]
        )
        if DataKey.EDGE_INDEX in data:
            from ._nequip import ensure_graph

            built_here = DataKey.AMD_ROWPTR not in data
            csr_err = ensure_graph(data, err=flags_dev[1:2]).get("_amd_csr_err")
            if not built_here and csr_err is not None:
                flags_dev[1:2] = csr_err
        order, seg, _ = ops.group_by_key(sidx, S, err=flags_dev[2:3])
        self._last_flags, self._last_Z = flags_dev, Z
        n_nodes = data[DataKey.POSITIONS].shape[0] if DataKey.POSITIONS in data else None
        if self.check_species == "deferred":
            self.finish_checks()
            host = torch.empty(3, dtype=torch.int32, pin_memory=True)
            host.copy_(flags_dev, non_blocking=True)
            ev = torch.cuda.Event()
            ev.record(torch.cuda.current_stream(Z.device))
            self._pending = (ev, host, Z, n_nodes)
        elif self.check_species:
            self.raise_for_last_flags(n_nodes)
        if not provided:
            data[DataKey.SPECIES_INDEX] = sidx
        data[DataKey.AMD_SPECIES] = (order, seg)
        data[DataKey.AMD_SPECIES_I32] = s32
        if attrs is not None:
            data[DataKey.NODE_ATTRS] = attrs
        if torch.is_grad_enabled() and self.linear.weight.requires_grad:
            from ..autograd import SpeciesEmbedFn

            if self.__dict__.get("_wgrad_segs") is None:
                from ._tables import DeviceTables

                dim = self.linear.weight.shape[0]
                self.__dict__["_wgrad_segs"] = DeviceTables(segs=np.array([[0, 1, 1, 0, dim, 0, 0, 0]], dtype=np.int32))
            feats = SpeciesEmbedFn.apply(self.linear.weight, self.linear.bias, feats, (order, seg),
                                         self._wgrad_segs.get("segs", feats.device))
        if self.use_atom_feats:
            extra = data["atom_feats"]
            if extra.dim() != 2 or extra.shape[0] != feats.shape[0]:
                raise ValueError(f"atom_feats must be [n_atoms, atom_feats_dim], got {tuple(extra.shape)}")
            feats = torch.cat([feats, extra.to(feats.dtype)], dim=1)
        data[DataKey.NODE_FEATURES] = feats
        return data


class EdgeLengthEmbedding(ModuleIrreps, torch.nn.Module):
    REQUIRED_KEYS_IRREPS_IN = [DataKey.POSITIONS, DataKey.EDGE_INDEX]

    def __init__(
        self,
        irreps_in: Dict[str, Irreps] = None,
        out_field: str = DataKey.EDGE_EMBEDDING,
        num_basis: int = 10,
        start: float = 0.0,
        end: float = 5.0,
        basis: str = "bessel",
        cutoff: bool = True,
        materialize: bool = False,
    ):
        super().__init__()
        if basis != "bessel" or not cutoff:
            raise NotImplementedError("matten_amd implements the Bessel basis with cutoff (all shipped configs)")
        self.num_basis, self.start, self.end, self.basis, self.cutoff = num_basis, start, end, basis, cutoff
        self.out_field = out_field
        self.materialize = materialize
        self.init_irreps(irreps_in, irreps_out={out_field: Irreps(f"{num_basis}x0e")})

    def forward(self, data: DataKey.Type) -> DataKey.Type:
        from ._nequip import ensure_edge_geometry

        data[DataKey.AMD_RBF] = torch.tensor([self.num_basis, self.start, self.end], dtype=torch.float64)
        if self.materialize:
            ensure_edge_geometry(data, want_lengths=True, want_embedding=True)
        return data
```

### matten_amd/ops.py

```python
from __future__ import annotations

from typing import Optional, Tuple

import os

import numpy as np

import torch

from . import _lib
from .nn._tables import bump_weights_epoch


_EVENTS = None
_EVENTS_ONLY = None


def enable_event_timing(flag: bool = True, only=None) -> None:
    global _EVENTS, _EVENTS_ONLY
    _EVENTS = {} if flag else None
    _EVENTS_ONLY = tuple(only) if (flag and only) else None


def event_timings_ms():
    if _EVENTS is None:
        return {}
    return {k: [a.elapsed_time(b) for a, b in v] for k, v in _EVENTS.items()}


class _timed:
    def __init__(self, name: str):
        self.name = name

    def __enter__(self):
        self.on = _EVENTS is not None and (_EVENTS_ONLY is None or self.name.startswith(_EVENTS_ONLY))
        if self.on:
            self.a = torch.cuda.Event(enable_timing=True)
            self.a.record(torch.cuda.current_stream())
        return self

    def __exit__(self, *exc):
        if self.on and _EVENTS is not None:
            b = torch.cuda.Event(enable_timing=True)
            b.record(torch.cuda.current_stream())
            _EVENTS.setdefault(self.name, []).append((self.a, b))
        return False


SH_STRIDE = 32


def _ptr(t: Optional[torch.Tensor]):
    return None if t is None else t.data_ptr()


_raw_stream = getattr(torch._C, "_cuda_getCurrentRawStream", None)


def _stream() -> int:
    if _raw_stream is not None:
        return _raw_stream(torch.cuda.current_device())
    return torch.cuda.current_stream().cuda_stream


def _need(t: torch.Tensor, dtype, name: str) -> torch.Tensor:
    if not isinstance(t, torch.Tensor):
        raise TypeError(f"{name}: expected a tensor, got {type(t)}")
    if not t.is_cuda:
        raise _lib.MattenHipError(
            f"{name} is on {t.device}: matten_amd runs on MI355X only (no CPU fallback). Move the batch to cuda."
        )
    if t.dtype != dtype:
        raise TypeError(f"{name}: expected dtype {dtype}, got {t.dtype}")
    return t if t.is_contiguous() else t.contiguous()


def _need_rows(t: torch.Tensor, dtype, name: str) -> torch.Tensor:
    if isinstance(t, torch.Tensor) and t.dim() == 2 and t.stride(1) == 1 and t.stride(0) >= t.shape[1] and t.is_cuda \
            and t.dtype == dtype:
        return t
    return _need(t, dtype, name)


def _err_flag(err, dev) -> torch.Tensor:
    if err is None:
        return torch.zeros(1, dtype=torch.int32, device=dev)
    if err.dtype != torch.int32 or err.numel() != 1 or err.device != dev:
        raise ValueError("err must be an int32 tensor of one element on the inputs' device")
    return err


def csr_build(edge_index: torch.Tensor, n_nodes: int, err: torch.Tensor = None) -> Tuple[torch.Tensor, torch.Tensor, torch.Tensor, torch.Tensor]:
    lib = _lib.load()
    edge_index = _need(edge_index, torch.int64, "edge_index")
    E = edge_index.shape[1]
    dev = edge_index.device
    perm = torch.empty(E, dtype=torch.int32, device=dev)
    rowptr = torch.empty(n_nodes + 1, dtype=torch.int32, device=dev)
    src = torch.empty(E, dtype=torch.int32, device=dev)
    err = _err_flag(err, dev)
    nbytes = lib.matten_csr_workspace_bytes(E, n_nodes)
    ws = torch.empty(max(nbytes, 1), dtype=torch.uint8, device=dev)
    _lib.check(
        lib.matten_csr_build(_ptr(edge_index), E, n_nodes, _ptr(perm), _ptr(rowptr), _ptr(src), _ptr(ws), nbytes,
                             _ptr(err), _stream()),
        "matten_csr_build",
    )
    return perm, rowptr, src, err


def csr_split(rowptr: torch.Tensor, n_edges: int, max_len: int, num_neigh: torch.Tensor = None):
    lib = _lib.load()
    rowptr = _need(rowptr, torch.int32, "rowptr")
    N = rowptr.shape[0] - 1
    bound = int(lib.matten_csr_split_bound(N, n_edges, max_len))
    dev = rowptr.device
    vrowptr = torch.empty(bound + 1, dtype=torch.int32, device=dev)
    vseg = torch.empty(N + 1, dtype=torch.int64, device=dev)
    vnn = None
    if num_neigh is not None:
        num_neigh = _need(num_neigh, torch.float32, "num_neigh")
        vnn = torch.empty(bound, dtype=torch.float32, device=dev)
    _lib.check(lib.matten_csr_split(_ptr(rowptr), N, n_edges, max_len, _ptr(vrowptr), _ptr(vseg), _ptr(num_neigh), _ptr(vnn),
                                    _stream()), "matten_csr_split")
    return vrowptr, vseg, vnn


def group_by_key(key: torch.Tensor, n_keys: int, err: torch.Tensor = None) -> Tuple[torch.Tensor, torch.Tensor, torch.Tensor]:
    lib = _lib.load()
    key = _need(key, torch.int64, "key")
    n = key.shape[0]
    dev = key.device
    order = torch.empty(n, dtype=torch.int32, device=dev)
    seg = torch.empty(n_keys + 1, dtype=torch.int32, device=dev)
    err = _err_flag(err, dev)
    nbytes = lib.matten_group_workspace_bytes(n, n_keys)
    ws = torch.empty(max(nbytes, 1), dtype=torch.uint8, device=dev)
    _lib.check(lib.matten_group_by_key(_ptr(key), n, n_keys, _ptr(order), _ptr(seg), _ptr(ws), nbytes, _ptr(err),
                                       _stream()), "matten_group_by_key")
    return order, seg, err


def species_embed(atomic_numbers, z_to_index, min_z: int, max_z: int, n_species: int, weight, bias,
                  want_attrs: bool = False, err: torch.Tensor = None):
    lib = _lib.load()
    Z = _need(atomic_numbers, torch.int64, "atomic_numbers")
    lut = _need(z_to_index, torch.int64, "_Z_to_index")
    W = _need(weight, torch.float32, "linear.weight")
    b = _need(bias, torch.float32, "linear.bias")
    N, dim = Z.shape[0], W.shape[0]
    dev = Z.device
    sidx = torch.empty(N, dtype=torch.int64, device=dev)
    s32 = torch.empty(N, dtype=torch.int32, device=dev)
    feats = torch.empty(N, dim, dtype=torch.float32, device=dev)
    attrs = torch.empty(N, n_species, dtype=torch.float32, device=dev) if want_attrs else None
    err = _err_flag(err, dev)
    _lib.check(
        lib.matten_species_embed(_ptr(Z), N, _ptr(lut), min_z, max_z, n_species, _ptr(W), _ptr(b), dim, _ptr(sidx),
                                 _ptr(s32), _ptr(feats), _ptr(attrs), _ptr(err), _stream()),
        "matten_species_embed",
    )
    return sidx, s32, feats, attrs, err


def edge_geom(pos, edge_index, edge_cell_shift, cell, batch, perm, lmax: int, n_basis: int = 0, r_start: float = 0.0,
              r_end: float = 1.0, want_vectors=False, want_lengths=False, want_attrs=False, want_embedding=False):
    lib = _lib.load()
    pos = _need(pos, torch.float32, "pos")
    edge_index = _need(edge_index, torch.int64, "edge_index")
    E = edge_index.shape[1]
    dev = pos.device
    n_cells = 0
    if cell is not None:
        cell = _need(cell, torch.float32, "cell").reshape(-1, 3, 3)
        n_cells = cell.shape[0]
        edge_cell_shift = _need(edge_cell_shift, torch.float32, "edge_cell_shift")
        if n_cells > 1:
            batch = _need(batch, torch.int64, "batch")
    sh_dim = (lmax + 1) ** 2
    geom = torch.empty(E, 4, dtype=torch.float32, device=dev)
    sh = torch.empty(E, SH_STRIDE, dtype=torch.float32, device=dev)
    out = {"geom_sorted": geom, "sh_sorted": sh}
    ev = torch.empty(E, 3, dtype=torch.float32, device=dev) if want_vectors else None
    el = torch.empty(E, dtype=torch.float32, device=dev) if want_lengths else None
    ea = torch.empty(E, sh_dim, dtype=torch.float32, device=dev) if want_attrs else None
    ee = torch.empty(E, n_basis, dtype=torch.float32, device=dev) if want_embedding else None
    _lib.check(
        lib.matten_edge_geom(_ptr(pos), _ptr(edge_index), _ptr(edge_cell_shift), _ptr(cell), n_cells, _ptr(batch),
                             _ptr(perm), E, pos.shape[0], lmax, n_basis, r_start, r_end, _ptr(geom), _ptr(sh), SH_STRIDE, _ptr(ev),
                             _ptr(el),
                             _ptr(ea), _ptr(ee), _stream()),
        "matten_edge_geom",
    )
    out.update(edge_vectors=ev, edge_lengths=el, edge_attrs=ea, edge_embedding=ee)
    return out


def _edge_dtype(t: torch.Tensor, name: str) -> torch.Tensor:
    if not isinstance(t, torch.Tensor) or t.dtype not in (torch.float32, torch.bfloat16):
        raise TypeError(f"{name}: expected an fp32 or bf16 tensor")
    return _need(t, t.dtype, name)


def radial_mlp(geom_sorted, n_basis: int, r_start: float, r_end: float, w0p, w1p, w2p, out_dtype=torch.float32) -> torch.Tensor:
    lib = _lib.load()
    geom_sorted = _need(geom_sorted, torch.float32, "geom_sorted")
    w0p, w1p, w2p = (_need(w, torch.float32, n) for w, n in ((w0p, "w0p"), (w1p, "w1p"), (w2p, "w2p")))
    E = geom_sorted.shape[0]
    nb_pad, hidden = w0p.shape
    w_pad = w2p.shape[1]
    if out_dtype not in (torch.float32, torch.bfloat16):
        raise TypeError("radial_mlp: out_dtype must be fp32 or bf16")
    out = torch.empty(E, w_pad, dtype=out_dtype, device=geom_sorted.device)
    with _timed(f"radial_mlp/w_pad={w_pad}"):
        rc = lib.matten_radial_mlp(_ptr(geom_sorted), E, n_basis, r_start, r_end, _ptr(w0p), nb_pad, _ptr(w1p),
                                   _ptr(w2p), hidden, w_pad, 1.0, _ptr(out), int(out_dtype == torch.bfloat16), _stream())
    _lib.check(rc, "matten_radial_mlp")
    return out


def radial_pack(w0, w1, w2, scales):
    lib = _lib.load()
    w0, w1, w2 = (_need(w, torch.float32, n) for w, n in ((w0, "layer0.weight"), (w1, "layer1.weight"), (w2, "layer2.weight")))
    nb, h = w0.shape
    W = w2.shape[1]
    nb_pad, w_pad = (nb + 3) // 4 * 4, (W + 15) // 16 * 16
    dev = w0.device
    w0p = torch.empty(nb_pad, h, dtype=torch.float32, device=dev)
    w1p = torch.empty(h, h, dtype=torch.float32, device=dev)
    w2p = torch.empty(h, w_pad, dtype=torch.float32, device=dev)
    _lib.check(lib.matten_radial_pack(_ptr(w0), _ptr(w1), _ptr(w2), nb, nb_pad, W, w_pad, float(scales[0]), float(scales[1]),
                                      float(scales[2]), _ptr(w0p), _ptr(w1p), _ptr(w2p), _stream()), "matten_radial_pack")
    return w0p, w1p, w2p


def fused_operands(w0, w1, w2, scales, cols, group_entries, n_tiles: int, r_start: float, r_end: float, act_cst: float):
    lib = _lib.load()
    w0, w1, w2 = (_need(w, torch.float32, n) for w, n in ((w0, "layer0.weight"), (w1, "layer1.weight"), (w2, "layer2.weight")))
    cols = _need(cols, torch.int64, "fused_cols")
    group_entries = _need(group_entries, torch.int32, "group_entries")
    nb, h = w0.shape
    W, n_cols = w2.shape[1], cols.numel()
    nb_pad, w_pad = (nb + 3) // 4 * 4, (n_cols + 15) // 16 * 16 + 16
    dev = w0.device
    w0p = torch.empty(nb_pad, h, dtype=torch.float32, device=dev)
    w1p = torch.empty(h, h, dtype=torch.float32, device=dev)
    w2p = torch.empty(h, w_pad, dtype=torch.float32, device=dev)
    hs = torch.empty(2, dtype=torch.float32, device=dev)
    n_ent = group_entries.shape[0]
    frag = torch.empty(n_tiles, 64, 16, dtype=torch.float16, device=dev)
    inv = torch.empty(n_ent, dtype=torch.float32, device=dev)
    st = _stream()
    _lib.check(lib.matten_radial_pack_cols(_ptr(w0), _ptr(w1), _ptr(w2), nb, nb_pad, W, _ptr(cols), n_cols, w_pad,
                                           float(scales[0]), float(scales[1]), float(scales[2]), _ptr(w0p), _ptr(w1p),
                                           _ptr(w2p), st), "matten_radial_pack_cols")
    _lib.check(lib.matten_radial_h_scale(_ptr(w0), _ptr(w1), nb, float(r_start), float(r_end), float(act_cst), _ptr(hs), st),
               "matten_radial_h_scale")
    _lib.check(lib.matten_split_a_tiles(_ptr(w2p), w_pad, _ptr(group_entries), n_ent, _ptr(hs), _ptr(frag), _ptr(inv), st),
               "matten_split_a_tiles")
    return w0p, w1p, w2p, hs, frag, inv


RADIAL_MAX_MID = 3


def _mid(w_mid, name: str):
    if not isinstance(w_mid, torch.Tensor) or w_mid.dim() != 3 or tuple(w_mid.shape[1:]) != (32, 32):
        raise ValueError(f"{name}: expected [n_mid, 32, 32]")
    n_mid = w_mid.shape[0]
    if n_mid > RADIAL_MAX_MID:
        raise ValueError(f"{name}: at most {RADIAL_MAX_MID} middle layers (invariant_layers <= {RADIAL_MAX_MID + 1})")
    return (_need(w_mid, torch.float32, name) if n_mid else None), n_mid


def radial_mlp_deep(geom_sorted, n_basis: int, r_start: float, r_end: float, w0p, w_mid, w2p,
                    out_dtype=torch.float32) -> torch.Tensor:
    lib = _lib.load()
    geom_sorted = _need(geom_sorted, torch.float32, "geom_sorted")
    w0p, w2p = _need(w0p, torch.float32, "w0p"), _need(w2p, torch.float32, "w2p")
    w_mid, n_mid = _mid(w_mid, "w_mid")
    E = geom_sorted.shape[0]
    nb_pad, hidden = w0p.shape
    w_pad = w2p.shape[1]
    if out_dtype not in (torch.float32, torch.bfloat16):
        raise TypeError("radial_mlp: out_dtype must be fp32 or bf16")
    out = torch.empty(E, w_pad, dtype=out_dtype, device=geom_sorted.device)
    with _timed(f"radial_mlp/w_pad={w_pad}"):
        rc = lib.matten_radial_mlp_deep(_ptr(geom_sorted), E, n_basis, r_start, r_end, _ptr(w0p), nb_pad, _ptr(w_mid), n_mid,
                                        _ptr(w2p), hidden, w_pad, 1.0, _ptr(out), int(out_dtype == torch.bfloat16), _stream())
    _lib.check(rc, "matten_radial_mlp_deep")
    return out


def radial_pack_deep(w0, w_mid, w2, scales):
    lib = _lib.load()
    w0, w2 = _need(w0, torch.float32, "layer0.weight"), _need(w2, torch.float32, "last layer weight")
    w_mid, n_mid = _mid(w_mid, "middle layer weights")
    nb, h = w0.shape
    W = w2.shape[1]
    nb_pad, w_pad = (nb + 3) // 4 * 4, (W + 15) // 16 * 16
    dev = w0.device
    w0p = torch.empty(nb_pad, h, dtype=torch.float32, device=dev)
    wmp = torch.empty(n_mid, h, h, dtype=torch.float32, device=dev)
    w2p = torch.empty(h, w_pad, dtype=torch.float32, device=dev)
    _lib.check(lib.matten_radial_pack_deep(_ptr(w0), _ptr(w_mid), n_mid, _ptr(w2), nb, nb_pad, W, w_pad, float(scales[0]),
                                           float(scales[1]), float(scales[2]), _ptr(w0p), _ptr(wmp) if n_mid else None,
                                           _ptr(w2p), _stream()), "matten_radial_pack_deep")
    return w0p, wmp, w2p


def radial_h_scale_deep(w0, w_mid, r_start: float, r_end: float, act_cst: float) -> torch.Tensor:
    lib = _lib.load()
    w0 = _need(w0, torch.float32, "layer0.weight")
    w_mid, n_mid = _mid(w_mid, "middle layer weights")
    hs = torch.empty(2, dtype=torch.float32, device=w0.device)
    _lib.check(lib.matten_radial_h_scale_deep(_ptr(w0), _ptr(w_mid), n_mid, w0.shape[0], float(r_start), float(r_end),
                                              float(act_cst), _ptr(hs), _stream()), "matten_radial_h_scale_deep")
    return hs


def fused_operands_deep(w0, w_mid, w2, scales, cols, group_entries, n_tiles: int, r_start: float, r_end: float,
                        act_cst: float):
    lib = _lib.load()
    w0, w2 = _need(w0, torch.float32, "layer0.weight"), _need(w2, torch.float32, "last layer weight")
    w_mid, n_mid = _mid(w_mid, "middle layer weights")
    cols = _need(cols, torch.int64, "fused_cols")
    group_entries = _need(group_entries, torch.int32, "group_entries")
    nb, h = w0.shape
    W, n_cols = w2.shape[1], cols.numel()
    nb_pad, w_pad = (nb + 3) // 4 * 4, (n_cols + 15) // 16 * 16 + 16
    dev = w0.device
    w0p = torch.empty(nb_pad, h, dtype=torch.float32, device=dev)
    wmp = torch.empty(n_mid, h, h, dtype=torch.float32, device=dev)
    w2p = torch.empty(h, w_pad, dtype=torch.float32, device=dev)
    hs = torch.empty(2, dtype=torch.float32, device=dev)
    n_ent = group_entries.shape[0]
    frag = torch.empty(n_tiles, 64, 16, dtype=torch.float16, device=dev)
    inv = torch.empty(n_ent, dtype=torch.float32, device=dev)
    st = _stream()
    _lib.check(lib.matten_radial_pack_cols_deep(_ptr(w0), _ptr(w_mid), n_mid, _ptr(w2), nb, nb_pad, W, _ptr(cols), n_cols,
                                                w_pad, float(scales[0]), float(scales[1]), float(scales[2]), _ptr(w0p),
                                                _ptr(wmp) if n_mid else None, _ptr(w2p), st), "matten_radial_pack_cols_deep")
    _lib.check(lib.matten_radial_h_scale_deep(_ptr(w0), _ptr(w_mid), n_mid, nb, float(r_start), float(r_end), float(act_cst),
                                              _ptr(hs), st), "matten_radial_h_scale_deep")
    _lib.check(lib.matten_split_a_tiles(_ptr(w2p), w_pad, _ptr(group_entries), n_ent, _ptr(hs), _ptr(frag), _ptr(inv), st),
               "matten_split_a_tiles")
    return w0p, wmp, w2p, hs, frag, inv


def radial_mlp_bwd_deep(geom_sorted, n_basis: int, r_start: float, r_end: float, w0p, w_mid, w2p, w_cols: int, dw,
                        scales=(1.0, 1.0, 1.0)):
    lib = _lib.load()
    geom_sorted = _need(geom_sorted, torch.float32, "geom_sorted")
    w0p, w2p = _need(w0p, torch.float32, "w0p"), _need(w2p, torch.float32, "w2p")
    w_mid, n_mid = _mid(w_mid, "w_mid")
    if dw.dtype not in (torch.float32, torch.bfloat16):
        raise TypeError("dw must be fp32 or bf16")
    dw = _need(dw, dw.dtype, "dw")
    E = geom_sorted.shape[0]
    nb_pad, hidden = w0p.shape
    w_pad = w2p.shape[1]
    dev = geom_sorted.device
    small_len = nb_pad * hidden + n_mid * hidden * hidden
    if E == 0:
        return w0p.new_zeros(nb_pad, hidden), w0p.new_zeros(n_mid, hidden, hidden), w2p.new_zeros(hidden, w_pad)
    n_small, n_rng = lib.matten_radial_mlp_bwd_small_slices(E), lib.matten_radial_mlp_bwd_w2_ranges_deep(E, w_pad, n_mid)
    h2 = torch.empty(E, hidden, dtype=torch.float32, device=dev)
    part_small = torch.empty(max(n_small, 1), small_len, dtype=torch.float32, device=dev)
    part_w2 = torch.empty(max(n_rng, 1), hidden, w_pad, dtype=torch.float32, device=dev)
    small = torch.empty(small_len, dtype=torch.float32, device=dev)
    d2 = torch.empty(hidden, w_pad, dtype=torch.float32, device=dev)
    with _timed(f"radial_mlp_bwd/w_pad={w_pad}"):
        rc = lib.matten_radial_mlp_bwd_deep(_ptr(geom_sorted), E, n_basis, r_start, r_end, _ptr(w0p), nb_pad, _ptr(w_mid),
                                            n_mid, _ptr(w2p), hidden, w_pad, int(w_cols), _ptr(dw), dw.shape[1],
                                            int(dw.dtype == torch.bfloat16), _ptr(h2), _ptr(part_small), _ptr(part_w2),
                                            float(scales[0]), float(scales[1]), float(scales[2]), _ptr(small), _ptr(d2),
                                            _stream())
    _lib.check(rc, "matten_radial_mlp_bwd_deep")
    return small[: nb_pad * hidden].reshape(nb_pad, hidden), small[nb_pad * hidden:].reshape(n_mid, hidden, hidden), d2


def gather_scale(src, idx, scale, scale_by_source: bool = False, perm2=None):
    lib = _lib.load()
    src = _need(src, torch.float32, "src")
    idx = _need(idx, torch.int64, "idx")
    scale = _need(scale, torch.float32, "scale")
    out = torch.empty(idx.shape, dtype=torch.float32, device=src.device)
    out2 = None
    if perm2 is not None:
        perm2 = _need(perm2, torch.int64, "perm2")
        out2 = torch.empty(idx.shape, dtype=torch.float32, device=src.device)
    _lib.check(lib.matten_gather_scale(_ptr(src), _ptr(idx), _ptr(scale), idx.numel(), scale.numel(), int(scale_by_source),
                                       _ptr(out), _ptr(perm2), _ptr(out2), _stream()), "matten_gather_scale")
    return out if perm2 is None else (out, out2)


def radial_mlp_bwd(geom_sorted, n_basis: int, r_start: float, r_end: float, w0p, w1p, w2p, w_cols: int, dw,
                   scales=(1.0, 1.0, 1.0)):
    lib = _lib.load()
    geom_sorted = _need(geom_sorted, torch.float32, "geom_sorted")
    w0p, w1p, w2p = (_need(w, torch.float32, n) for w, n in ((w0p, "w0p"), (w1p, "w1p"), (w2p, "w2p")))
    if dw.dtype not in (torch.float32, torch.bfloat16):
        raise TypeError("dw must be fp32 or bf16")
    dw = _need(dw, dw.dtype, "dw")
    E = geom_sorted.shape[0]
    nb_pad, hidden = w0p.shape
    w_pad = w2p.shape[1]
    dev = geom_sorted.device
    n_small, n_rng = lib.matten_radial_mlp_bwd_small_slices(E), lib.matten_radial_mlp_bwd_w2_ranges(E, w_pad)
    h2 = torch.empty(E, hidden, dtype=torch.float32, device=dev)
    part_small = torch.empty(max(n_small, 1), nb_pad * hidden + hidden * hidden, dtype=torch.float32, device=dev)
    part_w2 = torch.empty(max(n_rng, 1), hidden, w_pad, dtype=torch.float32, device=dev)
    if E == 0:
        return w0p.new_zeros(nb_pad, hidden), w1p.new_zeros(hidden, hidden), w2p.new_zeros(hidden, w_pad)
    small = torch.empty(nb_pad * hidden + hidden * hidden, dtype=torch.float32, device=dev)
    d2 = torch.empty(hidden, w_pad, dtype=torch.float32, device=dev)
    with _timed(f"radial_mlp_bwd/w_pad={w_pad}"):
        rc = lib.matten_radial_mlp_bwd(_ptr(geom_sorted), E, n_basis, r_start, r_end, _ptr(w0p), nb_pad, _ptr(w1p),
                                       _ptr(w2p), hidden, w_pad, int(w_cols), _ptr(dw), dw.shape[1],
                                       int(dw.dtype == torch.bfloat16), _ptr(h2), _ptr(part_small), _ptr(part_w2),
                                       float(scales[0]), float(scales[1]), float(scales[2]), _ptr(small), _ptr(d2),
                                       _stream())
    _lib.check(rc, "matten_radial_mlp_bwd")
    return small[: nb_pad * hidden].reshape(nb_pad, hidden), small[nb_pad * hidden:].reshape(hidden, hidden), d2


def tp_paths(x, w_edge, sh_sorted, rowptr, src_sorted, entries, unit_start, units_per_tile: int, d_mid: int,
             avg_num_neighbors: float, num_neigh=None) -> torch.Tensor:
    lib = _lib.load()
    from .plan import TP_TILE_NODES

    if lib.matten_tp_tile_nodes() != TP_TILE_NODES:
        raise _lib.MattenHipError("plan.TP_TILE_NODES does not match the library's node tile")
    x = _need(x, torch.float32, "node_features")
    w_edge = _edge_dtype(w_edge, "w_edge")
    sh_sorted = _need(sh_sorted, torch.float32, "sh_sorted")
    N, d_in = rowptr.shape[0] - 1, x.shape[1]
    if num_neigh is not None:
        num_neigh = _need(num_neigh, torch.float32, "num_neigh")
    agg = torch.empty(N, d_mid, dtype=torch.float32, device=x.device)
    with _timed(f"tp_scatter/d_mid={d_mid}"):
        rc = lib.matten_tp_paths(_ptr(x), d_in, _ptr(w_edge), w_edge.shape[1], _ptr(sh_sorted), sh_sorted.shape[1],
                                 _ptr(rowptr), _ptr(src_sorted), N, _ptr(entries), _ptr(unit_start),
                                 entries.shape[0], units_per_tile, d_mid, float(avg_num_neighbors or 0.0),
                                 _ptr(num_neigh), _ptr(agg), int(w_edge.dtype == torch.bfloat16), _stream())
    _lib.check(rc, "matten_tp_paths")
    return agg


def split_hidden(h2p: torch.Tensor) -> torch.Tensor:
    tiny = 2.0 ** -14
    hi = torch.where(h2p.abs() < tiny, torch.zeros_like(h2p), h2p.half().float())
    lo = (h2p - hi) * 2048.0
    lo = torch.where(lo.abs() < tiny, torch.zeros_like(lo), lo)
    return torch.stack([hi.half(), lo.half()], dim=1).contiguous()


def radial_hidden(geom_sorted, n_basis: int, r_start: float, r_end: float, w0p, w1p, h_scale=None) -> torch.Tensor:
    lib = _lib.load()
    geom_sorted = _need(geom_sorted, torch.float32, "geom_sorted")
    w0p, w1p = _need(w0p, torch.float32, "w0p"), _need(w1p, torch.float32, "w1p")
    E = geom_sorted.shape[0]
    h2p = torch.empty(E, 2, 32, dtype=torch.float16, device=geom_sorted.device)
    with _timed("radial_hidden"):
        if h_scale is not None:
            h_scale = _need(h_scale, torch.float32, "h_scale")
        rc = lib.matten_radial_hidden(_ptr(geom_sorted), E, n_basis, r_start, r_end, _ptr(w0p), w0p.shape[0],
                                      _ptr(w1p), w0p.shape[1], _ptr(h2p), _ptr(h_scale), _stream())
    _lib.check(rc, "matten_radial_hidden")
    return h2p


def radial_hidden_multi(geom_sorted, n_basis: int, r_start: float, r_end: float, w0ps, w1ps, h_scales=None):
    import ctypes

    lib = _lib.load()
    geom_sorted = _need(geom_sorted, torch.float32, "geom_sorted")
    w0ps = [_need(w, torch.float32, "w0p") for w in w0ps]
    w1ps = [_need(w, torch.float32, "w1p") for w in w1ps]
    L, E = len(w0ps), geom_sorted.shape[0]
    if not 1 <= L <= 8 or len(w1ps) != L or any(w.shape != w0ps[0].shape for w in w0ps):
        raise ValueError("radial_hidden_multi: 1..8 layers with equal basis / hidden sizes")
    out = [torch.empty(E, 2, 32, dtype=torch.float16, device=geom_sorted.device) for _ in range(L)]
    arr = lambda ts: (ctypes.c_void_p * L)(*[t.data_ptr() for t in ts])
    if h_scales is not None:
        h_scales = [_need(h, torch.float32, "h_scale") for h in h_scales]
        if len(h_scales) != L:
            raise ValueError("one h_scale per layer")
    with _timed("radial_hidden_multi"):
        rc = lib.matten_radial_hidden_multi(_ptr(geom_sorted), E, n_basis, r_start, r_end, arr(w0ps), w0ps[0].shape[0],
                                            arr(w1ps), w0ps[0].shape[1], arr(out),
                                            arr(h_scales) if h_scales is not None else None, L, _stream())
    _lib.check(rc, "matten_radial_hidden_multi")
    return out


def radial_hidden_deep(geom_sorted, n_basis: int, r_start: float, r_end: float, w0p, w_mid, h_scale=None) -> torch.Tensor:
    lib = _lib.load()
    geom_sorted = _need(geom_sorted, torch.float32, "geom_sorted")
    w0p = _need(w0p, torch.float32, "w0p")
    w_mid, n_mid = _mid(w_mid, "w_mid")
    E = geom_sorted.shape[0]
    h2p = torch.empty(E, 2, 32, dtype=torch.float16, device=geom_sorted.device)
    with _timed("radial_hidden"):
        if h_scale is not None:
            h_scale = _need(h_scale, torch.float32, "h_scale")
        rc = lib.matten_radial_hidden_deep(_ptr(geom_sorted), E, n_basis, r_start, r_end, _ptr(w0p), w0p.shape[0],
                                           _ptr(w_mid), n_mid, w0p.shape[1], _ptr(h2p), _ptr(h_scale), _stream())
    _lib.check(rc, "matten_radial_hidden_deep")
    return h2p


def radial_hidden_multi_deep(geom_sorted, n_basis: int, r_start: float, r_end: float, w0ps, w_mids, h_scales=None):
    import ctypes

    lib = _lib.load()
    geom_sorted = _need(geom_sorted, torch.float32, "geom_sorted")
    w0ps = [_need(w, torch.float32, "w0p") for w in w0ps]
    mids = [_mid(w, "w_mid") for w in w_mids]
    L, E = len(w0ps), geom_sorted.shape[0]
    if not 1 <= L <= 8 or len(mids) != L or any(w.shape != w0ps[0].shape for w in w0ps) or \
            any(m[1] != mids[0][1] for m in mids):
        raise ValueError("radial_hidden_multi_deep: 1..8 layers with equal basis / hidden sizes and depth")
    n_mid = mids[0][1]
    out = [torch.empty(E, 2, 32, dtype=torch.float16, device=geom_sorted.device) for _ in range(L)]
    arr = lambda ts: (ctypes.c_void_p * L)(*[t.data_ptr() for t in ts])
    if h_scales is not None:
        h_scales = [_need(h, torch.float32, "h_scale") for h in h_scales]
        if len(h_scales) != L:
            raise ValueError("one h_scale per layer")
    with _timed("radial_hidden_multi"):
        rc = lib.matten_radial_hidden_multi_deep(_ptr(geom_sorted), E, n_basis, r_start, r_end, arr(w0ps), w0ps[0].shape[0],
                                                 arr([m[0] for m in mids]) if n_mid else None, n_mid, w0ps[0].shape[1],
                                                 arr(out), arr(h_scales) if h_scales is not None else None, L, _stream())
    _lib.check(rc, "matten_radial_hidden_multi_deep")
    return out


def split_a_tiles(w2p: torch.Tensor, group_entries) -> Tuple[torch.Tensor, torch.Tensor]:
    dev = w2p.device
    g = torch.arange(4, device=dev)[:, None]
    kk = torch.arange(8, device=dev)[None, :]
    k_idx = 16 * (kk >> 2) + 4 * g + (kk & 3)
    tiny = 2.0 ** -14
    tiles, inv = [], []
    for row in np.asarray(group_entries).reshape(-1, 32):
        w_base, n_mt = int(row[5]), int(row[7])
        if int(row[0]) < 0 or n_mt == 0:
            inv.append(torch.ones((), device=dev))
            continue
        A = w2p[k_idx][:, :, w_base:w_base + 16 * n_mt]
        A = A.reshape(4, 8, n_mt, 16).permute(2, 0, 3, 1)
        amax = A.abs().max()
        e = torch.where(amax > 0, (torch.frexp(amax)[1] - 1).clamp(-100, 100), torch.full_like(amax, 13, dtype=torch.int32))
        scale = torch.ldexp(torch.ones_like(amax), 13 - e)
        inv.append(torch.ldexp(torch.ones_like(amax), e - 13))
        v = A * scale
        hi = torch.where(v.abs() < tiny, torch.zeros_like(v), v.half().float())
        lo = (v - hi) * 2048.0
        lo = torch.where(lo.abs() < tiny, torch.zeros_like(lo), lo)
        tiles.append(torch.cat([hi.half(), lo.half()], dim=-1).reshape(n_mt, 64, 16))
    return torch.cat(tiles).contiguous(), torch.stack(inv).float().contiguous()


_GROUPS_CHECKED = False


def tp_fused(x, h2p, w2p, sh_sorted, rowptr, src_sorted, entries, unit_map, units_per_tile: int,
             lds_floats_per_wave: int, d_mid: int, avg_num_neighbors: float, num_neigh=None,
             a_split=None) -> torch.Tensor:
    lib = _lib.load()
    from .plan import TP_TILE_NODES

    if lib.matten_tp_tile_nodes() != TP_TILE_NODES:
        raise _lib.MattenHipError("plan.TP_TILE_NODES does not match the library's node tile")
    from .plan import TP_MAX_COLS, TP_MAX_COLS_L0, TP_MAX_COLS_L1
    if (lib.matten_tp_max_cols() != TP_MAX_COLS or lib.matten_tp_max_cols_l0() != TP_MAX_COLS_L0
            or lib.matten_tp_max_cols_l1() != TP_MAX_COLS_L1):
        raise _lib.MattenHipError("plan.TP_MAX_COLS does not match the library's entry width (-DTPF_MAX_COLS)")
    global _GROUPS_CHECKED
    from .plan import tp_groups_hash
    if not _GROUPS_CHECKED and lib.matten_tp_groups_hash() != tp_groups_hash():
        raise _lib.MattenHipError("the library's coupling code (cg_gen.h) was generated for other coupling groups than plan.TP_GROUPS "
                                  "(MATTEN_TP_GROUPS / an interrupted tools/*.sh A/B build?): make -C matten_amd/csrc clean all")
    _GROUPS_CHECKED = True
    x = _need_rows(x, torch.float32, "node_features")
    h2p = _need(h2p, torch.float16, "h2s")
    if h2p.dim() != 3 or h2p.shape[1:] != (2, 32):
        raise ValueError(f"h2s must be [E,2,32] fp16 (ops.split_hidden / ops.radial_hidden), got {tuple(h2p.shape)}")
    w2p = _need(w2p, torch.float32, "w2p")
    sh_sorted = _need(sh_sorted, torch.float32, "sh_sorted")
    N, d_in = rowptr.shape[0] - 1, x.stride(0)
    if num_neigh is not None:
        num_neigh = _need(num_neigh, torch.float32, "num_neigh")
    if a_split is not None:
        a_split = (_need(a_split[0], torch.float16, "a_split"), _need(a_split[1], torch.float32, "a_scale_inv"))
        if a_split[1].numel() != entries.shape[0]:
            raise ValueError("a_scale_inv needs one value per group entry")
    if unit_map.numel() != units_per_tile:
        raise ValueError(f"unit_map has {unit_map.numel()} units, expected {units_per_tile} (plan.fused_unit_map)")
    agg = torch.empty(N, d_mid, dtype=torch.float32, device=x.device)
    with _timed(f"tp_scatter/d_mid={d_mid}/d_in={x.shape[1]}"):
        rc = lib.matten_tp_fused(_ptr(x), d_in, _ptr(h2p), _ptr(w2p), w2p.shape[1], _ptr(sh_sorted),
                                 sh_sorted.shape[1], _ptr(rowptr), _ptr(src_sorted), N, _ptr(entries),
                                 _ptr(unit_map), entries.shape[0], units_per_tile, lds_floats_per_wave, d_mid,
                                 float(avg_num_neighbors or 0.0), _ptr(num_neigh),
                                 _ptr(a_split[0]) if a_split is not None else None,
                                 _ptr(a_split[1]) if a_split is not None else None, _ptr(agg), _stream())
    _lib.check(rc, "matten_tp_fused")
    return agg


def agg_linear(agg, species_order, wtab, io_table, blocks, d_out: int, add=None) -> torch.Tensor:
    lib = _lib.load()
    from .plan import AGG_BLOCK, AGG_MAX_MT
    if lib.matten_agg_linear_block_chunks() != AGG_BLOCK or lib.matten_agg_linear_max_mt() != AGG_MAX_MT:
        raise _lib.MattenHipError("plan.AGG_BLOCK / AGG_MAX_MT do not match the library (-DAL_BLK_CHUNKS)")
    agg = _need(agg, torch.float32, "agg")
    wtab = _need(wtab, torch.float32, "A fragments")
    n_rows, ld = agg.shape
    order, seg = species_order if species_order is not None else (None, None)
    n_species = wtab.shape[0] if wtab.dim() == 2 else 1
    if add is not None:
        add = _need_rows(add, torch.float32, "add")
    out = torch.empty(n_rows, d_out, dtype=torch.float32, device=agg.device)
    with _timed(f"agg_linear/ld={ld}"):
        rc = lib.matten_agg_linear(_ptr(agg), ld, _ptr(order), _ptr(seg), n_species, _ptr(wtab), wtab.shape[-1],
                                   _ptr(io_table), io_table.shape[0], _ptr(blocks), blocks.shape[0], _ptr(add),
                                   add.stride(0) if add is not None else d_out, d_out, n_rows, _ptr(out), _stream())
    _lib.check(rc, "matten_agg_linear")
    return out


def agg_linear_gate(agg, species_order, wtab, io_table, blocks, d_out: int, cmeta, act_cst, d_act: int, add=None,
                    bn_scale=None, bn_shift=None) -> torch.Tensor:
    lib = _lib.load()
    from .plan import AGG_BLOCK, AGG_GATE_SETS, AGG_MAX_MT
    if (lib.matten_agg_linear_block_chunks() != AGG_BLOCK or lib.matten_agg_linear_max_mt() != AGG_MAX_MT
            or lib.matten_agg_linear_gate_sets() != AGG_GATE_SETS):
        raise _lib.MattenHipError("plan.AGG_BLOCK / AGG_MAX_MT / AGG_GATE_SETS do not match the library")
    agg = _need(agg, torch.float32, "agg")
    wtab = _need(wtab, torch.float32, "A fragments")
    n_rows, ld = agg.shape
    order, seg = species_order if species_order is not None else (None, None)
    n_species = wtab.shape[0] if wtab.dim() == 2 else 1
    if add is not None:
        add = _need_rows(add, torch.float32, "add")
    if cmeta.shape != (d_out, 4):
        raise ValueError("cmeta must be [d_out, 4]")
    if bn_scale is not None:
        bn_scale, bn_shift = _need(bn_scale, torch.float32, "bn_scale"), _need(bn_shift, torch.float32, "bn_shift")
        if bn_scale.numel() != d_act or bn_shift.numel() != d_act:
            raise ValueError("bn_scale / bn_shift must have one value per activated column")
    out = torch.empty(n_rows, d_act, dtype=torch.float32, device=agg.device)
    with _timed(f"agg_linear/ld={ld}"):
        rc = lib.matten_agg_linear_gate(_ptr(agg), ld, _ptr(order), _ptr(seg), n_species, _ptr(wtab), wtab.shape[-1],
                                        _ptr(io_table), io_table.shape[0], _ptr(blocks), blocks.shape[0], _ptr(add),
                                        add.stride(0) if add is not None else d_out, d_out, n_rows, _ptr(cmeta),
                                        _ptr(act_cst), _ptr(bn_scale), _ptr(bn_shift), d_act, _ptr(out), _stream())
    _lib.check(rc, "matten_agg_linear_gate")
    return out


_SL_ROWS_LDS_BYTES = 52 * 1024


def species_linear(x, species_order, wp, w_stride: int, item_tables, d_out: int, add=None,
                   fully_covered: bool = True, variant: Optional[str] = None) -> torch.Tensor:
    lib = _lib.load()
    x = _need(x, torch.float32, "x")
    from . import selfcheck
    selfcheck.check_species_linear(x.device)
    wp = _need(wp, torch.float32, "packed weights")
    n_rows, d_in = x.shape
    order, seg = species_order if species_order is not None else (None, None)
    n_species = wp.shape[0] if wp.dim() == 2 else 1
    cur_add = add
    if cur_add is not None:
        cur_add = _need_rows(cur_add, torch.float32, "add")
    if fully_covered:
        out = torch.empty(n_rows, d_out, dtype=torch.float32, device=x.device)
    else:
        out = cur_add.clone() if cur_add is not None else torch.zeros(n_rows, d_out, dtype=torch.float32, device=x.device)
    rows_fits = len(item_tables) == 1 and 4 * (16 * (d_in | 1) + w_stride + 8 * item_tables[0].shape[0] + 4) <= _SL_ROWS_LDS_BYTES
    rows_variant = rows_fits and os.environ.get("MATTEN_SL_ROWS", "1") != "0"
    if variant is not None:
        rows_variant = rows_fits and variant == "rows"
    for items in item_tables:
        fn = lib.matten_species_linear_rows if rows_variant else lib.matten_species_linear
        _lib.check(
            fn(_ptr(x), d_in, _ptr(order), _ptr(seg), n_species, _ptr(wp), w_stride,
                                      _ptr(items), items.shape[0], d_out, _ptr(cur_add),
                                      cur_add.stride(0) if cur_add is not None else d_out, n_rows, _ptr(out), _stream()),
            "matten_species_linear",
        )
        cur_add = out
    return out


def gate_bn(x, meta, act_cst, running_mean=None, running_var=None, bn_weight=None, bn_bias=None, eps: float = 1e-5):
    lib = _lib.load()
    x = _need(x, torch.float32, "x")
    n_rows, d_in = x.shape
    d_out = meta.shape[0]
    out = torch.empty(n_rows, d_out, dtype=torch.float32, device=x.device)
    _lib.check(
        lib.matten_gate_bn(_ptr(x), d_in, _ptr(meta), d_out, _ptr(act_cst), _ptr(running_mean), _ptr(running_var),
                           _ptr(bn_weight), _ptr(bn_bias), eps, n_rows, _ptr(out), _stream()),
        "matten_gate_bn",
    )
    return out


def segment_reduce(x, ptr, mean: bool) -> torch.Tensor:
    lib = _lib.load()
    x = _need(x, torch.float32, "x")
    ptr = _need(ptr, torch.int64, "ptr")
    B = ptr.shape[0] - 1
    out = torch.empty(B, x.shape[1], dtype=torch.float32, device=x.device)
    _lib.check(lib.matten_segment_reduce(_ptr(x), x.shape[1], _ptr(ptr), B, int(mean), _ptr(out), _stream()),
               "matten_segment_reduce")
    return out


def segment_minmax(x, ptr, take_max: bool, want_arg: bool = False):
    lib = _lib.load()
    x = _need(x, torch.float32, "x")
    ptr = _need(ptr, torch.int64, "ptr")
    B = ptr.shape[0] - 1
    out = torch.empty(B, x.shape[1], dtype=torch.float32, device=x.device)
    arg = torch.empty(B, x.shape[1], dtype=torch.int64, device=x.device) if want_arg else None
    _lib.check(lib.matten_segment_minmax(_ptr(x), x.shape[1], _ptr(ptr), B, int(take_max), _ptr(out), _ptr(arg), _stream()),
               "matten_segment_minmax")
    return (out, arg) if want_arg else out


def segment_minmax_bwd(dy, arg, n_rows: int) -> torch.Tensor:
    lib = _lib.load()
    dy = _need(dy, torch.float32, "dy")
    dx = torch.zeros(n_rows, dy.shape[1], dtype=torch.float32, device=dy.device)
    _lib.check(lib.matten_segment_minmax_bwd(_ptr(dy), dy.shape[1], _ptr(arg), dy.shape[0], _ptr(dx), _stream()),
               "matten_segment_minmax_bwd")
    return dx


def dense_rows(x, q) -> torch.Tensor:
    lib = _lib.load()
    x = _need(x, torch.float32, "x")
    q = _need(q, torch.float32, "q")
    out = torch.empty(x.shape[0], q.shape[1], dtype=torch.float32, device=x.device)
    _lib.check(lib.matten_dense_rows(_ptr(x), x.shape[1], _ptr(q), q.shape[1], x.shape[0], _ptr(out), _stream()),
               "matten_dense_rows")
    return out


def tp_backward(x, w_edge, sh_sorted, src_sorted, dst_sorted, col_meta, nnz_ijk, nnz_c, g_agg,
                avg_num_neighbors: float, num_neigh=None, in_groups=None):
    lib = _lib.load()
    x = _need(x, torch.float32, "x")
    w_edge = _edge_dtype(w_edge, "w_edge")
    g_agg = _need(g_agg, torch.float32, "grad agg")
    N, d_in = x.shape
    E = w_edge.shape[0]
    W = col_meta.shape[0]
    dx = torch.zeros(N, d_in, dtype=torch.float32, device=x.device)
    dw = torch.empty(E, w_edge.shape[1], dtype=w_edge.dtype, device=x.device)
    if num_neigh is not None:
        num_neigh = _need(num_neigh, torch.float32, "num_neigh")
    with _timed(f"tp_backward/d_mid={g_agg.shape[1]}/d_in={d_in}"):
        rc = lib.matten_tp_backward(_ptr(x), d_in, _ptr(w_edge), w_edge.shape[1], _ptr(sh_sorted), sh_sorted.shape[1],
                                    _ptr(src_sorted), _ptr(dst_sorted), _ptr(col_meta), W, _ptr(nnz_ijk), _ptr(nnz_c),
                                    _ptr(g_agg), g_agg.shape[1], float(avg_num_neighbors or 0.0), _ptr(num_neigh), E,
                                    _ptr(dx), _ptr(dw), dw.shape[1], _ptr(in_groups[0]) if in_groups else None,
                                    _ptr(in_groups[1]) if in_groups else None,
                                    in_groups[0].shape[0] - 1 if in_groups else 0,
                                    int(w_edge.dtype == torch.bfloat16), _stream())
    _lib.check(rc, "matten_tp_backward")
    return dx, dw


def split_a_tiles_dev(w2p, entries, n_tiles: int, h_scale=None):
    lib = _lib.load()
    w2p = _need(w2p, torch.float32, "w2p")
    entries = _need(entries, torch.int32, "entries")
    frag = torch.empty(n_tiles, 64, 16, dtype=torch.float16, device=w2p.device)
    inv = torch.empty(entries.shape[0], dtype=torch.float32, device=w2p.device)
    _lib.check(lib.matten_split_a_tiles(_ptr(w2p), w2p.shape[1], _ptr(entries), entries.shape[0], _ptr(h_scale), _ptr(frag),
                                        _ptr(inv), _stream()), "matten_split_a_tiles")
    return frag, inv


WFREE_MAX_MUL = 256


def tp_backward_lit(x, w_edge, sh_sorted, src_sorted, dst_sorted, blocks, paths, sum_lanes: int, g_agg,
                    avg_num_neighbors: float, num_neigh=None, out_csr=None, blocks_cover_input: bool = True, wfree=None,
                    dw_shape=None, lds_floats: int = 4096, max_l: int = 4, max_mul: int = 256):
    lib = _lib.load()
    x = _need(x, torch.float32, "x")
    g_agg = _need(g_agg, torch.float32, "grad agg")
    N, d_in = x.shape
    if wfree is not None:
        if w_edge is not None or dw_shape is None:
            raise ValueError("wfree: pass w_edge=None and dw_shape=((E, ld), dtype)")
        h2s, frag, w_inv = (_need(t, dt, n) for t, dt, n in zip(wfree, (torch.float16, torch.float16, torch.float32),
                                                                ("h2s", "frag", "w_inv")))
        (E, dw_ld), dw_dtype = dw_shape
        if h2s.shape != (E, 2, 32) or w_inv.numel() != paths.shape[0]:
            raise ValueError("wfree: h2s must be [E, 2, 32] and w_inv hold one value per path")
    else:
        w_edge = _edge_dtype(w_edge, "w_edge")
        E, dw_ld, dw_dtype = w_edge.shape[0], w_edge.shape[1], w_edge.dtype
    if out_csr is not None:
        out_ptr, out_perm = (_need(t, torch.int32, n) for t, n in zip(out_csr, ("out_ptr", "out_perm")))
        dx = torch.empty(N, d_in, dtype=torch.float32, device=x.device)
        dx_edges = (torch.empty if blocks_cover_input else torch.zeros)(E, d_in, dtype=torch.float32, device=x.device)
    else:
        out_ptr = out_perm = dx_edges = None
        dx = torch.zeros(N, d_in, dtype=torch.float32, device=x.device)
    dw = torch.empty(E, dw_ld, dtype=dw_dtype, device=x.device)
    if num_neigh is not None:
        num_neigh = _need(num_neigh, torch.float32, "num_neigh")
    if wfree is not None:
        with _timed(f"tp_backward/d_mid={g_agg.shape[1]}/d_in={d_in}"):
            rc = lib.matten_tp_backward_lit_wfree(_ptr(x), d_in, _ptr(h2s), _ptr(frag), _ptr(w_inv), _ptr(sh_sorted),
                                                  sh_sorted.shape[1], _ptr(src_sorted), _ptr(dst_sorted), _ptr(blocks),
                                                  blocks.shape[0], int(sum_lanes), _ptr(paths), paths.shape[0], _ptr(g_agg),
                                                  g_agg.shape[1], float(avg_num_neighbors or 0.0), _ptr(num_neigh), E, _ptr(dx),
                                                  _ptr(dw), dw_ld, int(dw_dtype == torch.bfloat16), N, _ptr(out_ptr),
                                                  _ptr(out_perm), _ptr(dx_edges), int(lds_floats), int(max_l), int(max_mul),
                                                  _stream())
        _lib.check(rc, "matten_tp_backward_lit_wfree")
        return dx, dw
    with _timed(f"tp_backward/d_mid={g_agg.shape[1]}/d_in={d_in}"):
        rc = lib.matten_tp_backward_lit(_ptr(x), d_in, _ptr(w_edge), w_edge.shape[1], _ptr(sh_sorted), sh_sorted.shape[1],
                                        _ptr(src_sorted), _ptr(dst_sorted), _ptr(blocks), blocks.shape[0], int(sum_lanes),
                                        _ptr(paths), paths.shape[0], _ptr(g_agg), g_agg.shape[1],
                                        float(avg_num_neighbors or 0.0), _ptr(num_neigh), E, _ptr(dx), _ptr(dw),
                                        dw.shape[1], int(w_edge.dtype == torch.bfloat16), N, _ptr(out_ptr), _ptr(out_perm),
                                        _ptr(dx_edges), int(max_l), _stream())
    _lib.check(rc, "matten_tp_backward_lit")
    return dx, dw


def species_linear_wgrad(x, dy, species_order, n_species: int, seg_tables, w_stride: int) -> torch.Tensor:
    lib = _lib.load()
    x = _need(x, torch.float32, "x")
    dy = _need(dy, torch.float32, "dy")
    order, seg = species_order if species_order is not None else (None, None)
    n_scratch = lib.matten_species_linear_wgrad_scratch_floats(x.shape[0], n_species, w_stride)
    dwp = torch.empty(n_species, w_stride, dtype=torch.float32, device=x.device)
    partial = torch.empty(n_scratch, dtype=torch.float32, device=x.device) if n_scratch > 0 else None
    for segs in seg_tables:
        _lib.check(
            lib.matten_species_linear_wgrad(_ptr(x), x.shape[1], _ptr(dy), dy.shape[1], _ptr(order), _ptr(seg),
                                            n_species, x.shape[0], _ptr(segs), segs.shape[0], w_stride, _ptr(dwp),
                                            _ptr(partial), _stream()),
            "matten_species_linear_wgrad",
        )
    return dwp


def gate_bwd(x, meta, act_cst, dy) -> torch.Tensor:
    lib = _lib.load()
    x = _need(x, torch.float32, "x")
    dy = _need(dy, torch.float32, "dy")
    dx = torch.empty_like(x)
    _lib.check(lib.matten_gate_bwd(_ptr(x), x.shape[1], _ptr(meta), meta.shape[0], _ptr(act_cst), _ptr(dy), x.shape[0],
                                   _ptr(dx), _stream()), "matten_gate_bwd")
    return dx


def _bn_scratch(lib, x):
    n = lib.matten_bn_scratch_floats(x.shape[0], x.shape[1])
    return torch.empty(n, dtype=torch.float32, device=x.device) if n > 0 else None


def bn_train_fwd(x, col2chan, chan, weight, bias, eps: float, running_mean=None, running_var=None, momentum: float = 0.0):
    lib = _lib.load()
    x = _need(x, torch.float32, "x")
    C = chan.shape[0]
    mean = torch.empty(C, dtype=torch.float32, device=x.device)
    nu = torch.empty(C, dtype=torch.float32, device=x.device)
    y = torch.empty_like(x)
    if running_var is not None:
        running_mean = _need(running_mean, torch.float32, "running_mean")
        running_var = _need(running_var, torch.float32, "running_var")
    scratch = _bn_scratch(lib, x)
    _lib.check(lib.matten_bn_train_fwd(_ptr(x), x.shape[1], x.shape[0], _ptr(col2chan), _ptr(chan), C, _ptr(weight),
                                       _ptr(bias), eps, _ptr(mean), _ptr(nu), _ptr(y), _ptr(running_mean),
                                       _ptr(running_var), float(momentum), _ptr(scratch), _stream()),
               "matten_bn_train_fwd")
    if running_var is not None:
        bump_weights_epoch()
    return y, mean, nu


def norm_act(x, chan, act: int, epsilon: float = 1e-8, running_mean=None, running_var=None, bn_weight=None, bn_bias=None,
             bn_eps: float = 1e-5) -> torch.Tensor:
    lib = _lib.load()
    x = _need(x, torch.float32, "x")
    y = torch.empty_like(x)
    _lib.check(lib.matten_norm_act(_ptr(x), x.shape[1], x.shape[0], _ptr(chan), chan.shape[0], int(act), float(epsilon),
                                   _ptr(running_mean), _ptr(running_var), _ptr(bn_weight), _ptr(bn_bias), float(bn_eps),
                                   _ptr(y), _stream()), "matten_norm_act")
    return y


def norm_act_bwd(x, dy, chan, act: int, epsilon: float = 1e-8) -> torch.Tensor:
    lib = _lib.load()
    dy = _need(dy, torch.float32, "dy")
    dx = torch.empty_like(x)
    _lib.check(lib.matten_norm_act_bwd(_ptr(x), _ptr(dy), x.shape[1], x.shape[0], _ptr(chan), chan.shape[0], int(act),
                                       float(epsilon), _ptr(dx), _stream()), "matten_norm_act_bwd")
    return dx


def instance_norm_fwd(x, seg_ptr, seg_of_row, col2chan, chan, weight, bias, eps: float):
    lib = _lib.load()
    x = _need(x, torch.float32, "x")
    seg_ptr = _need(seg_ptr, torch.int64, "ptr")
    seg_of_row = _need(seg_of_row, torch.int64, "batch")
    C, B = chan.shape[0], seg_ptr.shape[0] - 1
    mean = torch.empty(B, C, dtype=torch.float32, device=x.device)
    nu = torch.empty(B, C, dtype=torch.float32, device=x.device)
    y = torch.empty_like(x)
    _lib.check(lib.matten_instance_norm_fwd(_ptr(x), x.shape[1], x.shape[0], _ptr(seg_ptr), _ptr(seg_of_row), B,
                                            _ptr(col2chan), _ptr(chan), C, _ptr(weight), _ptr(bias), eps, _ptr(mean),
                                            _ptr(nu), _ptr(y), _stream()), "matten_instance_norm_fwd")
    return y, mean, nu


def instance_norm_bwd(x, dy, seg_ptr, seg_of_row, col2chan, chan, mean, nu, weight, eps: float):
    lib = _lib.load()
    dy = _need(dy, torch.float32, "dy")
    B, C = mean.shape
    A = torch.empty(B, C, dtype=torch.float32, device=x.device)
    Bs = torch.empty(B, C, dtype=torch.float32, device=x.device)
    dx = torch.empty_like(x)
    _lib.check(lib.matten_instance_norm_bwd(_ptr(x), _ptr(dy), x.shape[1], x.shape[0], _ptr(seg_ptr), _ptr(seg_of_row), B,
                                            _ptr(col2chan), _ptr(chan), C, _ptr(mean), _ptr(nu), _ptr(weight), eps,
                                            _ptr(A), _ptr(Bs), _ptr(dx), _stream()), "matten_instance_norm_bwd")
    return dx, A, Bs


def bn_train_bwd(x, dy, col2chan, chan, mean, nu, weight, eps: float, n_bias: int):
    lib = _lib.load()
    dy = _need(dy, torch.float32, "dy")
    C = chan.shape[0]
    A = torch.empty(C, dtype=torch.float32, device=x.device)
    B = torch.empty(C, dtype=torch.float32, device=x.device)
    dweight = torch.empty(C, dtype=torch.float32, device=x.device)
    dbias = torch.empty(n_bias, dtype=torch.float32, device=x.device)
    dx = torch.empty_like(x)
    scratch = _bn_scratch(lib, x)
    _lib.check(lib.matten_bn_train_bwd(_ptr(x), _ptr(dy), x.shape[1], x.shape[0], _ptr(col2chan), _ptr(chan), C,
                                       _ptr(mean), _ptr(nu), _ptr(weight), eps, _ptr(A), _ptr(B), _ptr(dx), _ptr(dweight),
                                       _ptr(dbias), _ptr(scratch), _stream()),
               "matten_bn_train_bwd")
    return dx, dweight, dbias


def segment_reduce_bwd(dy, ptr, n_rows: int, mean: bool) -> torch.Tensor:
    lib = _lib.load()
    dy = _need(dy, torch.float32, "dy")
    ptr = _need(ptr, torch.int64, "ptr")
    dx = torch.zeros(n_rows, dy.shape[1], dtype=torch.float32, device=dy.device)
    _lib.check(lib.matten_segment_reduce_bwd(_ptr(dy), dy.shape[1], _ptr(ptr), dy.shape[0], int(mean), _ptr(dx),
                                             _stream()), "matten_segment_reduce_bwd")
    return dx


def graph_prep(pos64, cell64, ptr, r_cut: float):
    lib = _lib.load()
    pos64 = _need(pos64, torch.float64, "pos")
    cell64 = _need(cell64, torch.float64, "cell")
    ptr = _need(ptr, torch.int64, "ptr")
    N, B, dev = pos64.shape[0], ptr.shape[0] - 1, pos64.device
    frac = torch.empty(N, 3, dtype=torch.float64, device=dev)
    bound = torch.empty(B, 3, dtype=torch.float64, device=dev)
    batch = torch.empty(N, dtype=torch.int64, device=dev)
    pos32 = torch.empty(N, 3, dtype=torch.float32, device=dev)
    cell32 = torch.empty(3 * B, 3, dtype=torch.float32, device=dev)
    _lib.check(lib.matten_graph_prep(_ptr(pos64), _ptr(cell64), _ptr(ptr), B, float(r_cut), _ptr(frac), _ptr(bound),
                                     _ptr(batch), _ptr(pos32), _ptr(cell32), _stream()), "matten_graph_prep")
    return frac, bound, batch, pos32, cell32


def neighbor_list(pos64, cell64, ptr, frac, bound, pair_ptr, r_cut: float, max_atoms: int, n_pairs: int, want_csr: bool = True):
    lib = _lib.load()
    pos64 = _need(pos64, torch.float64, "pos")
    cell64 = _need(cell64, torch.float64, "cell")
    ptr = _need(ptr, torch.int64, "ptr")
    frac = _need(frac, torch.float64, "frac")
    bound = _need(bound, torch.float64, "bound")
    pair_ptr = _need(pair_ptr, torch.int64, "pair_ptr")
    B = ptr.shape[0] - 1
    N = pos64.shape[0]
    dev = pos64.device
    counts = torch.empty((2 if want_csr else 1) * n_pairs, dtype=torch.int32, device=dev)
    with _timed("neighbor_count"):
        _lib.check(
            lib.matten_neighbor_count(_ptr(pos64), _ptr(cell64), _ptr(ptr), _ptr(frac), _ptr(bound), _ptr(pair_ptr),
                                      float(r_cut), B, int(max_atoms), _ptr(counts),
                                      counts.data_ptr() + 4 * n_pairs if (want_csr and n_pairs) else None, _stream()),
            "matten_neighbor_count",
        )
    scan = torch.zeros(counts.numel() + 1, dtype=torch.int64, device=dev)
    torch.cumsum(counts, 0, dtype=torch.int64, out=scan[1:])
    offsets = scan[: n_pairs + 1]
    if n_pairs:
        summary = torch.empty(2, dtype=torch.int64, device=dev)
        _lib.check(lib.matten_neighbor_summary(_ptr(offsets), _ptr(pair_ptr), B, _ptr(summary), _stream()),
                   "matten_neighbor_summary")
        E, min_edges = summary.tolist()
    else:
        E, min_edges = 0, 0
    edge_index = torch.empty(2, E, dtype=torch.int64, device=dev)
    shifts = torch.empty(E, 3, dtype=torch.float32, device=dev)
    num_neigh = torch.empty(N, dtype=torch.float32, device=dev)
    csr = offsets_t = None
    if want_csr and n_pairs and E < 2 ** 31:
        offsets_t = scan[n_pairs:]
        csr = (torch.empty(E, dtype=torch.int32, device=dev), torch.empty(N + 1, dtype=torch.int32, device=dev),
               torch.empty(E, dtype=torch.int32, device=dev))
    with _timed("neighbor_fill"):
        _lib.check(
            lib.matten_neighbor_fill(_ptr(pos64), _ptr(cell64), _ptr(ptr), _ptr(frac), _ptr(bound), _ptr(pair_ptr),
                                     float(r_cut), B, int(max_atoms), _ptr(offsets), E, _ptr(edge_index), _ptr(shifts),
                                     _ptr(num_neigh), _ptr(offsets_t), N, _ptr(csr[1]) if csr else None,
                                     _ptr(csr[2]) if csr else None, _ptr(csr[0]) if csr else None, _stream()),
            "matten_neighbor_fill",
        )
    return edge_index, shifts, num_neigh, offsets, int(min_edges), csr
```

Measured before the change: 1.241 billion edge-TP/s.

## Fold species embedding into first conv's lin1 and self-connection tables

Since the first conv layer's input features depend only on species, the lin1 and self-connection outputs are precomputed per species into a table. The embedding kernel then gathers these rows directly. When the aggregation linear runs in species-sorted mode, the self-connection addend is read per species instead of per row. This removes the first layer's lin1 and self-connection matmuls and the per-node addend traffic. In exchange it adds a cached derived table, new kernel variants and another code path that only applies in inference without gradients.

```diff
diff --git a/include/matten_hip.h b/include/matten_hip.h
--- a/include/matten_hip.h
+++ b/include/matten_hip.h
@@ -37,6 +37,11 @@
                          int64_t min_z, int64_t max_z, int64_t n_species, const float* weight ,
                          const float* bias , int64_t dim, int64_t* species_index, int32_t* species_i32,
                          float* node_feats, float* node_attrs, int32_t* err_flag, matten_stream_t stream);
+int matten_species_embed_rows(const int64_t* atomic_numbers, int64_t n_nodes, const int64_t* z_to_index,
+                              int64_t min_z, int64_t max_z, int64_t n_species, const float* weight ,
+                              const float* bias , int64_t dim, const float* table, int64_t table_ld,
+                              int64_t rows_dim, int64_t* species_index, int32_t* species_i32, float* node_feats,
+                              float* rows, float* node_attrs, int32_t* err_flag, matten_stream_t stream);
 
 int matten_edge_geom(const float* pos, const int64_t* edge_index, const float* edge_cell_shift,
                      const float* cell, int64_t n_cells, const int64_t* batch, const int32_t* perm,
@@ -72,6 +77,12 @@
                            int64_t n_rows, const int32_t* cmeta, const float* act_cst, const float* bn_scale,
                            const float* bn_shift, int64_t d_act, float* out, matten_stream_t stream);
 int matten_agg_linear_gate_sets(void);
+int matten_agg_linear_species_add(const float* agg, int64_t ld, const int32_t* order, const int32_t* seg,
+                                  int64_t n_species, const float* wtab, int64_t w_stride, const int32_t* io_table,
+                                  int64_t n_io, const int32_t* blocks, int64_t n_blocks, const float* add,
+                                  int64_t add_ld, int64_t d_out, int64_t n_rows, const int32_t* cmeta,
+                                  const float* act_cst, const float* bn_scale, const float* bn_shift, int64_t d_act,
+                                  float* out, matten_stream_t stream);
 int matten_radial_hidden(const float* geom_sorted, int64_t n_edges, int n_basis, float r_start, float r_end,
                          const float* w0p, int nb_pad, const float* w1p, int hidden, uint16_t* h2s,
                          const float* h_scale, matten_stream_t stream);
diff --git a/matten_amd/_lib.py b/matten_amd/_lib.py
--- a/matten_amd/_lib.py
+++ b/matten_amd/_lib.py
@@ -7,7 +7,7 @@
 _HERE = os.path.dirname(os.path.abspath(__file__))
 LIB_PATH = os.path.join(_HERE, "libmatten_hip.so")
 
-ABI_VERSION = 45
+ABI_VERSION = 46
 
 P = c_void_p
 SIGNATURES = {
@@ -20,6 +20,8 @@
     "matten_csr_split": (c_int, [P, c_int64, c_int64, c_int64, P, P, P, P, P]),
     "matten_group_by_key": (c_int, [P, c_int64, c_int64, P, P, P, c_size_t, P, P]),
     "matten_species_embed": (c_int, [P, c_int64, P, c_int64, c_int64, c_int64, P, P, c_int64, P, P, P, P, P, P]),
+    "matten_species_embed_rows": (c_int, [P, c_int64, P, c_int64, c_int64, c_int64, P, P, c_int64, P, c_int64, c_int64, P,
+                                          P, P, P, P, P, P]),
     "matten_edge_geom": (c_int, [P, P, P, P, c_int64, P, P, c_int64, c_int64, c_int, c_int, c_float, c_float, P, P, c_int, P, P, P, P, P]),
     "matten_radial_mlp": (c_int, [P, c_int64, c_int, c_float, c_float, P, c_int, P, P, c_int, c_int, c_float, P, c_int, P]),
     "matten_radial_mlp_deep": (c_int, [P, c_int64, c_int, c_float, c_float, P, c_int, P, c_int, P, c_int, c_int, c_float, P, c_int,
@@ -38,6 +40,8 @@
     "matten_agg_linear_gate": (c_int, [P, c_int64, P, P, c_int64, P, c_int64, P, c_int64, P, c_int64, P, c_int64, c_int64,
                                        c_int64, P, P, P, P, c_int64, P, P]),
     "matten_agg_linear_gate_sets": (c_int, []),
+    "matten_agg_linear_species_add": (c_int, [P, c_int64, P, P, c_int64, P, c_int64, P, c_int64, P, c_int64, P, c_int64,
+                                              c_int64, c_int64, P, P, P, P, c_int64, P, P]),
     "matten_radial_hidden": (c_int, [P, c_int64, c_int, c_float, c_float, P, c_int, P, c_int, P, P, P]),
     "matten_radial_hidden_deep": (c_int, [P, c_int64, c_int, c_float, c_float, P, c_int, P, c_int, c_int, P, P, P]),
     "matten_tp_max_cols": (c_int, []),
diff --git a/matten_amd/csrc/agg_linear.hip b/matten_amd/csrc/agg_linear.hip
--- a/matten_amd/csrc/agg_linear.hip
+++ b/matten_amd/csrc/agg_linear.hip
@@ -70,7 +70,7 @@
 #else
 #define AL_OCC
 #endif
-template <bool GATE>
+template <bool GATE, bool SPECIES_ADD>
 __global__ __launch_bounds__(AL_WAVES * 64, AL_MIN_BLOCKS) AL_OCC void agg_linear_kernel(Args a) {
     extern __shared__ __attribute__((aligned(16))) float lds[];
     AggIo* io_l = reinterpret_cast<AggIo*>(lds + a.w_stride);
@@ -166,7 +166,7 @@
         ocol = out_off + fv * d3 + k0 + (fc - fv * kk);
 #pragma unroll
         for (int p = 0; p < 8; ++p) {
-            const int rid = max(rowid[2 * p + frow], 0);
+            const int rid = SPECIES_ADD ? s : max(rowid[2 * p + frow], 0);
             addv[p] = has_add ? a.add[(int64_t)rid * a.add_ld + ocol] : 0.0f;
         }
         if constexpr (GATE && AL_GATE_PREFETCH) {
@@ -340,7 +340,7 @@
                              const float* wtab, int64_t w_stride, const int32_t* io_table, int64_t n_io,
                              const int32_t* blocks, int64_t n_blocks, const float* add, int64_t add_ld, int64_t d_out,
                              int64_t n_rows, float* out, const int32_t* cmeta, const float* act_cst, const float* bn_scale,
-                             const float* bn_shift, int64_t out_ld, hipStream_t stream) {
+                             const float* bn_shift, int64_t out_ld, bool add_species, hipStream_t stream) {
     if (n_rows < 0 || ld <= 0 || (ld & 3) || n_species <= 0 || w_stride <= 0 || (w_stride & 3) || n_io <= 0 ||
         n_blocks <= 0 || d_out <= 0 || out_ld <= 0)
         return MATTEN_EINVAL;
@@ -349,6 +349,7 @@
     if ((order == nullptr) != (seg == nullptr)) return MATTEN_EINVAL;
     if (!order && n_species != 1) return MATTEN_EINVAL;
     if (add && add_ld < d_out) return MATTEN_EINVAL;
+    if (add_species && !add) return MATTEN_EINVAL;
     if (cmeta && !act_cst) return MATTEN_EINVAL;
     if ((bn_scale == nullptr) != (bn_shift == nullptr)) return MATTEN_EINVAL;
     const size_t lds = matten_agg_linear_lds_bytes(w_stride, n_io, n_blocks);
@@ -359,21 +360,26 @@
         if (hipGetDevice(&dev) != hipSuccess || dev < 0) return MATTEN_ELAUNCH;
         const uint64_t bit = dev < 64 ? (uint64_t)1 << dev : 0;
         if (!bit || !(raised.load(std::memory_order_acquire) & bit)) {
-            if (hipFuncSetAttribute((const void*)agg_linear_kernel<false>, hipFuncAttributeMaxDynamicSharedMemorySize,
-                                    (int)AL_MAX_LDS) != hipSuccess ||
-                hipFuncSetAttribute((const void*)agg_linear_kernel<true>, hipFuncAttributeMaxDynamicSharedMemorySize,
-                                    (int)AL_MAX_LDS) != hipSuccess)
-                return MATTEN_ELAUNCH;
+            const void* fns[] = {(const void*)agg_linear_kernel<false, false>, (const void*)agg_linear_kernel<true, false>,
+                                 (const void*)agg_linear_kernel<false, true>, (const void*)agg_linear_kernel<true, true>};
+            for (const void* fn : fns)
+                if (hipFuncSetAttribute(fn, hipFuncAttributeMaxDynamicSharedMemorySize, (int)AL_MAX_LDS) != hipSuccess)
+                    return MATTEN_ELAUNCH;
             raised.fetch_or(bit, std::memory_order_release);
         }
     }
     const int64_t grid = matten_cdiv(n_rows, AL_WAVES * AL_ROWS) + n_species;
     if (grid >= ((int64_t)1 << 31) || n_rows >= ((int64_t)1 << 31)) return MATTEN_EINVAL;
     Args a{agg, order, seg, wtab, (const AggIo*)io_table, (const AggBlk*)blocks, add, out, ld, (int)n_species,
-           (int)w_stride, (int)n_io, (int)n_blocks, (int)add_ld, (int)d_out, (int)n_rows, (const int4*)cmeta, act_cst,
-           bn_scale, bn_shift, (int)out_ld};
-    if (cmeta) agg_linear_kernel<true><<<(unsigned)grid, AL_WAVES * 64, lds, stream>>>(a);
-    else agg_linear_kernel<false><<<(unsigned)grid, AL_WAVES * 64, lds, stream>>>(a);
+           (int)w_stride, (int)n_io, (int)n_blocks, (int)add_ld, (int)d_out, (int)n_rows, (const int4*)cmeta,
+           act_cst, bn_scale, bn_shift, (int)out_ld};
+    if (add_species) {
+        if (cmeta) agg_linear_kernel<true, true><<<(unsigned)grid, AL_WAVES * 64, lds, stream>>>(a);
+        else agg_linear_kernel<false, true><<<(unsigned)grid, AL_WAVES * 64, lds, stream>>>(a);
+    } else {
+        if (cmeta) agg_linear_kernel<true, false><<<(unsigned)grid, AL_WAVES * 64, lds, stream>>>(a);
+        else agg_linear_kernel<false, false><<<(unsigned)grid, AL_WAVES * 64, lds, stream>>>(a);
+    }
     MATTEN_LAUNCH_CHECK();
     return MATTEN_OK;
 }
@@ -383,7 +389,7 @@
                                  int64_t n_io, const int32_t* blocks, int64_t n_blocks, const float* add,
                                  int64_t add_ld, int64_t d_out, int64_t n_rows, float* out, matten_stream_t stream_) {
     return agg_linear_launch(agg, ld, order, seg, n_species, wtab, w_stride, io_table, n_io, blocks, n_blocks, add, add_ld,
-                             d_out, n_rows, out, nullptr, nullptr, nullptr, nullptr, d_out, (hipStream_t)stream_);
+                             d_out, n_rows, out, nullptr, nullptr, nullptr, nullptr, d_out, false, (hipStream_t)stream_);
 }
 
 extern "C" int matten_agg_linear_gate_sets(void) { return AL_GATE_SETS; }
@@ -396,5 +402,18 @@
                                       float* out, matten_stream_t stream_) {
     if (!cmeta || d_act <= 0) return MATTEN_EINVAL;
     return agg_linear_launch(agg, ld, order, seg, n_species, wtab, w_stride, io_table, n_io, blocks, n_blocks, add, add_ld,
-                             d_out, n_rows, out, cmeta, act_cst, bn_scale, bn_shift, d_act, (hipStream_t)stream_);
-}
+                             d_out, n_rows, out, cmeta, act_cst, bn_scale, bn_shift, d_act, false, (hipStream_t)stream_);
+}
+
+extern "C" int matten_agg_linear_species_add(const float* agg, int64_t ld, const int32_t* order, const int32_t* seg,
+                                             int64_t n_species, const float* wtab, int64_t w_stride,
+                                             const int32_t* io_table, int64_t n_io, const int32_t* blocks,
+                                             int64_t n_blocks, const float* add, int64_t add_ld, int64_t d_out,
+                                             int64_t n_rows, const int32_t* cmeta, const float* act_cst,
+                                             const float* bn_scale, const float* bn_shift, int64_t d_act, float* out,
+                                             matten_stream_t stream_) {
+    if (!add || (cmeta && d_act <= 0)) return MATTEN_EINVAL;
+    return agg_linear_launch(agg, ld, order, seg, n_species, wtab, w_stride, io_table, n_io, blocks, n_blocks, add, add_ld,
+                             d_out, n_rows, out, cmeta, act_cst, bn_scale, bn_shift, cmeta ? d_act : d_out, true,
+                             (hipStream_t)stream_);
+}
diff --git a/matten_amd/csrc/edge.hip b/matten_amd/csrc/edge.hip
--- a/matten_amd/csrc/edge.hip
+++ b/matten_amd/csrc/edge.hip
@@ -85,11 +85,13 @@
     }
 }
 
+template <bool ROWS>
 __global__ void species_embed_kernel(const int64_t* __restrict__ Z, int64_t N, const int64_t* __restrict__ lut,
                                      int64_t min_z, int64_t max_z, int64_t S, const float* __restrict__ W,
-                                     const float* __restrict__ b, int64_t dim, int64_t* __restrict__ species_index,
+                                     const float* __restrict__ b, int64_t dim, const float* __restrict__ table,
+                                     int64_t table_ld, int64_t rows_dim, int64_t* __restrict__ species_index,
                                      int32_t* __restrict__ species_i32, float* __restrict__ feats,
-                                     float* __restrict__ attrs, int32_t* err_flag) {
+                                     float* __restrict__ rows, float* __restrict__ attrs, int32_t* err_flag) {
     int64_t n = (int64_t)blockIdx.x * blockDim.y + threadIdx.y;
     if (n >= N) return;
     int64_t z = Z[n];
@@ -109,6 +111,8 @@
     }
     int64_t s = idx < 0 ? 0 : idx;
     for (int64_t d = threadIdx.x; d < dim; d += blockDim.x) feats[n * dim + d] = W[d * S + s] + b[d];
+    if (ROWS)
+        for (int64_t d = threadIdx.x; d < rows_dim; d += blockDim.x) rows[n * rows_dim + d] = table[s * table_ld + d];
     if (attrs)
         for (int64_t c = threadIdx.x; c < S; c += blockDim.x) attrs[n * S + c] = (c == idx) ? 1.0f : 0.0f;
 }
@@ -125,9 +129,28 @@
     if (n_nodes == 0) return MATTEN_OK;
     if (!atomic_numbers || !z_to_index || !weight || !bias || !node_feats || !err_flag) return MATTEN_EINVAL;
     dim3 block(16, 16);
-    species_embed_kernel<<<(unsigned)matten_cdiv(n_nodes, 16), block, 0, stream>>>(
-        atomic_numbers, n_nodes, z_to_index, min_z, max_z, n_species, weight, bias, dim, species_index, species_i32,
-        node_feats, node_attrs, err_flag);
+    species_embed_kernel<false><<<(unsigned)matten_cdiv(n_nodes, 16), block, 0, stream>>>(
+        atomic_numbers, n_nodes, z_to_index, min_z, max_z, n_species, weight, bias, dim, nullptr, 0, 0, species_index,
+        species_i32, node_feats, nullptr, node_attrs, err_flag);
+    MATTEN_LAUNCH_CHECK();
+    return MATTEN_OK;
+}
+
+extern "C" int matten_species_embed_rows(const int64_t* atomic_numbers, int64_t n_nodes, const int64_t* z_to_index,
+                                         int64_t min_z, int64_t max_z, int64_t n_species, const float* weight,
+                                         const float* bias, int64_t dim, const float* table, int64_t table_ld,
+                                         int64_t rows_dim, int64_t* species_index, int32_t* species_i32,
+                                         float* node_feats, float* rows, float* node_attrs, int32_t* err_flag,
+                                         matten_stream_t stream_) {
+    hipStream_t stream = (hipStream_t)stream_;
+    if (n_nodes < 0 || dim <= 0 || n_species <= 0 || rows_dim <= 0 || table_ld < rows_dim) return MATTEN_EINVAL;
+    if (n_nodes == 0) return MATTEN_OK;
+    if (!atomic_numbers || !z_to_index || !weight || !bias || !table || !node_feats || !rows || !err_flag)
+        return MATTEN_EINVAL;
+    dim3 block(16, 16);
+    species_embed_kernel<true><<<(unsigned)matten_cdiv(n_nodes, 16), block, 0, stream>>>(
+        atomic_numbers, n_nodes, z_to_index, min_z, max_z, n_species, weight, bias, dim, table, table_ld, rows_dim,
+        species_index, species_i32, node_feats, rows, node_attrs, err_flag);
     MATTEN_LAUNCH_CHECK();
     return MATTEN_OK;
 }
diff --git a/matten_amd/csrc/node.hip b/matten_amd/csrc/node.hip
--- a/matten_amd/csrc/node.hip
+++ b/matten_amd/csrc/node.hip
@@ -197,4 +197,4 @@
     return MATTEN_OK;
 }
 
-extern "C" int matten_abi_version(void) { return 45; }
+extern "C" int matten_abi_version(void) { return 46; }
diff --git a/matten_amd/model_factory/tfn_scalar_tensor.py b/matten_amd/model_factory/tfn_scalar_tensor.py
--- a/matten_amd/model_factory/tfn_scalar_tensor.py
+++ b/matten_amd/model_factory/tfn_scalar_tensor.py
@@ -77,7 +77,21 @@
     backbone = create_sequential_module(modules=layers)
     link_radial_mlps(backbone)
     eliminate_dead_outputs(backbone)
+    fold_species_embedding(backbone)
     return backbone
+
+
+def fold_species_embedding(backbone) -> None:
+    from ..data.irreps import DataKey
+
+    mods = list(backbone._modules.values())
+    for i, emb in enumerate(mods):
+        if type(emb) is not SpeciesEmbedding or DataKey.NODE_FEATURES not in emb.out_fields:
+            continue
+        rest = [m for m in mods[i + 1:] if not isinstance(m, (SphericalHarmonicEdgeAttrs, EdgeLengthEmbedding))]
+        if rest and type(rest[0]) in (PointConv, PointConvWithActivation):
+            emb.__dict__["_lin1_sc_into"] = rest[0].conv if type(rest[0]) is PointConvWithActivation else rest[0]
+        return
 
 
 def eliminate_dead_outputs(backbone) -> None:
diff --git a/matten_amd/nn/conv.py b/matten_amd/nn/conv.py
--- a/matten_amd/nn/conv.py
+++ b/matten_amd/nn/conv.py
@@ -19,6 +19,8 @@
 KEPT_ONLY = "_amd_kept_irreps_only"
 DEAD_PATH_ELIMINATION = _os.environ.get("MATTEN_DEAD_PATH_ELIMINATION", "1") != "0"
 AGG_KM_MIN_ROWS = int(_os.environ.get("MATTEN_AGG_KM_MIN_ROWS", "8192"))
+LIN1_SC_READY = "_amd_lin1_sc_ready"
+LIN1_FUSE = _os.environ.get("MATTEN_LIN1_FUSE", "1") != "0"
 
 
 class PointConv(ModuleIrreps, torch.nn.Module):
@@ -67,6 +69,27 @@
                                                 scale=ap.scale)
                 self._agg_wtab = DerivedWeight(self._pack_agg_weights)
 
+    def takes_species_rows(self, n_rows: int) -> bool:
+        return self.agg_plan is not None and n_rows >= AGG_KM_MIN_ROWS
+
+    def species_lin1_sc(self, emb_weight: torch.Tensor, emb_bias: torch.Tensor):
+        if not self._fused_lin1_sc_tables():
+            return None
+        cache = self.__dict__.get("_species_lin1_sc")
+        if cache is None:
+            cache = self.__dict__["_species_lin1_sc"] = DerivedWeight(self._species_table)
+        return cache.get(emb_weight, emb_bias, self.lin1.weight, self.sc.weight)
+
+    def _species_table(self, we: torch.Tensor, be: torch.Tensor, w1: torch.Tensor, w2: torch.Tensor) -> torch.Tensor:
+        S, dev = we.shape[1], we.device
+        ids = torch.arange(S, dtype=torch.int64, device=dev)
+        x0 = ops.species_embed(ids, ids, 0, S - 1, S, we, be)[2]
+        species = (ids.to(torch.int32), torch.arange(S + 1, dtype=torch.int32, device=dev))
+        d1, d2 = self.lin1.plan.d_out, self.sc.plan.d_out
+        return ops.species_linear(x0, species, self._lin1_sc_packed.get(w1, w2),
+                                  self.lin1.plan.w_stride + self.sc.plan.w_stride,
+                                  [self._fused_lin1_sc_tables().get("meta", dev)], d1 + d2)
+
     def _pack_lin1_sc(self, w1: torch.Tensor, w2: torch.Tensor) -> torch.Tensor:
         return torch.cat([self.lin1._pack(w1), self.sc._pack(w2)], dim=1).contiguous()
 
@@ -151,15 +174,23 @@
                     mod.__dict__["weight"] = None
 
     def forward(self, data: DataKey.Type) -> DataKey.Type:
+        ready = data.pop(LIN1_SC_READY, None)
+        if ready is not None and ready[0] is not self:
+            raise RuntimeError("the species embedding prepared lin1 + self-connection for another conv layer")
         if self._view is not None and DEAD_PATH_ELIMINATION:
+            if ready is not None:
+                raise RuntimeError("lin1 + self-connection from species tables reached a dead-output view")
             data = self._view_forward(data, _ag.needs_grad_lazy(lambda: (data[DataKey.NODE_FEATURES], *_ag.params_of(self))))
             data[KEPT_ONLY] = True
             return data
         data.pop(KEPT_ONLY, None)
         x = data[DataKey.NODE_FEATURES]
         species = data[DataKey.AMD_SPECIES]
-        fused = None if _ag.needs_grad(x, self.lin1.weight, self.sc.weight) else self._fused_lin1_sc_tables()
-        if fused:
+        sc_species = False
+        fused = None if ready is not None or _ag.needs_grad(x, self.lin1.weight, self.sc.weight) else self._fused_lin1_sc_tables()
+        if ready is not None:
+            _, x1, self_connection, sc_species = ready
+        elif fused:
             wp = self._lin1_sc_packed.get(self.lin1.weight, self.sc.weight)
             d1, d2 = self.lin1.plan.d_out, self.sc.plan.d_out
             both = ops.species_linear(x, species, wp, self.lin1.plan.w_stride + self.sc.plan.w_stride,
@@ -177,13 +208,16 @@
                 cmeta, act_cst, d_act, bn_scale, bn_shift = gate
                 data[DataKey.NODE_FEATURES] = ops.agg_linear_gate(
                     agg, species, self._agg_wtab.get(self.lin2.weight), t.get("io", dev), t.get("blocks", dev), ap.d_out,
-                    cmeta, act_cst, d_act, add=self_connection, bn_scale=bn_scale, bn_shift=bn_shift)
+                    cmeta, act_cst, d_act, add=self_connection, bn_scale=bn_scale, bn_shift=bn_shift,
+                    add_species=sc_species)
                 data[GATE_APPLIED] = True
                 return data
             data[DataKey.NODE_FEATURES] = ops.agg_linear(agg, species, self._agg_wtab.get(self.lin2.weight),
                                                          t.get("io", dev), t.get("blocks", dev), ap.d_out,
-                                                         add=self_connection)
+                                                         add=self_connection, add_species=sc_species)
             return data
+        if sc_species:
+            raise RuntimeError("a per-species self-connection needs the streaming lin2 route")
         agg = self.tp(x1, data, self.avg_num_neighbors)
         data[DataKey.NODE_FEATURES] = self.lin2(agg, species, add=self_connection)
         return data
diff --git a/matten_amd/nn/embedding.py b/matten_amd/nn/embedding.py
--- a/matten_amd/nn/embedding.py
+++ b/matten_amd/nn/embedding.py
@@ -3,9 +3,11 @@
 import numpy as np
 import torch
 
+from .. import autograd as _ag
 from .. import ops
 from ..data.irreps import DataKey, ModuleIrreps
 from ..o3 import Irreps
+from . import conv as _conv
 
 
 class _AtomicNumberToIndex(torch.nn.Module):
@@ -86,6 +88,19 @@
         )
         self.linear = torch.nn.Linear(self.num_species, embedding_dim)
 
+    def _lin1_sc_fold(self, n_rows: int):
+        conv = self.__dict__.get("_lin1_sc_into")
+        if conv is None or not _conv.LIN1_FUSE or self.use_atom_feats or self.materialize:
+            return None
+        if conv._view is not None and _conv.DEAD_PATH_ELIMINATION:
+            return None
+        if _ag.needs_grad_lazy(lambda: (*_ag.params_of(self), *_ag.params_of(conv))):
+            return None
+        table = conv.species_lin1_sc(self.linear.weight, self.linear.bias)
+        if table is None:
+            return None
+        return conv, table, conv.takes_species_rows(n_rows)
+
     def finish_checks(self) -> None:
         pending, self._pending = getattr(self, "_pending", None), None
         if pending is None:
@@ -120,9 +135,19 @@
         else:
             raise ValueError("Nothing in `data` to encode. Need either species_index or atomic_numbers")
         flags_dev = torch.zeros(3, dtype=torch.int32, device=Z.device)
-        sidx, s32, feats, attrs, _ = ops.species_embed(
-            Z, lut, lo, hi, S, self.linear.weight, self.linear.bias, want_attrs=self.materialize, err=flags_dev[0:1]
-        )
+        fold = self._lin1_sc_fold(Z.shape[0])
+        data.pop(_conv.LIN1_SC_READY, None)
+        if fold is None:
+            sidx, s32, feats, attrs, _ = ops.species_embed(
+                Z, lut, lo, hi, S, self.linear.weight, self.linear.bias, want_attrs=self.materialize, err=flags_dev[0:1]
+            )
+        else:
+            conv, table, per_species = fold
+            d1 = conv.lin1.plan.d_out
+            sidx, s32, feats, rows, attrs, _ = ops.species_embed_rows(
+                Z, lut, lo, hi, S, self.linear.weight, self.linear.bias, table, d1 if per_species else table.shape[1],
+                want_attrs=self.materialize, err=flags_dev[0:1])
+            data[_conv.LIN1_SC_READY] = (conv, rows[:, :d1], table[:, d1:] if per_species else rows[:, d1:], per_species)
         if DataKey.EDGE_INDEX in data:
             from ._nequip import ensure_graph
 
diff --git a/matten_amd/ops.py b/matten_amd/ops.py
--- a/matten_amd/ops.py
+++ b/matten_amd/ops.py
@@ -161,6 +161,40 @@
         "matten_species_embed",
     )
     return sidx, s32, feats, attrs, err
+
+
+def species_embed_rows(atomic_numbers, z_to_index, min_z: int, max_z: int, n_species: int, weight, bias, table,
+                       rows_dim: int, want_attrs: bool = False, err: torch.Tensor = None):
+    lib = _lib.load()
+    Z = _need(atomic_numbers, torch.int64, "atomic_numbers")
+    lut = _need(z_to_index, torch.int64, "_Z_to_index")
+    W = _need(weight, torch.float32, "linear.weight")
+    b = _need(bias, torch.float32, "linear.bias")
+    T = _need_rows(table, torch.float32, "table")
+    if T.dim() != 2 or T.shape[0] != n_species or T.shape[1] < rows_dim:
+        raise ValueError(f"table must be [{n_species}, >= {rows_dim}], got {tuple(T.shape)}")
+    N, dim = Z.shape[0], W.shape[0]
+    dev = Z.device
+    sidx = torch.empty(N, dtype=torch.int64, device=dev)
+    s32 = torch.empty(N, dtype=torch.int32, device=dev)
+    feats = torch.empty(N, dim, dtype=torch.float32, device=dev)
+    rows = torch.empty(N, rows_dim, dtype=torch.float32, device=dev)
+    attrs = torch.empty(N, n_species, dtype=torch.float32, device=dev) if want_attrs else None
+    err = _err_flag(err, dev)
+    _lib.check(
+        lib.matten_species_embed_rows(_ptr(Z), N, _ptr(lut), min_z, max_z, n_species, _ptr(W), _ptr(b), dim, _ptr(T),
+                                      T.stride(0), rows_dim, _ptr(sidx), _ptr(s32), _ptr(feats), _ptr(rows),
+                                      _ptr(attrs), _ptr(err), _stream()),
+        "matten_species_embed_rows",
+    )
+    return sidx, s32, feats, rows, attrs, err
+
+
+def _species_add(add, n_species: int, d_out: int) -> torch.Tensor:
+    add = _need_rows(add, torch.float32, "add")
+    if add.dim() != 2 or add.shape[0] != n_species or add.shape[1] < d_out:
+        raise ValueError(f"a per-species addend must be [{n_species}, >= {d_out}], got {tuple(add.shape)}")
+    return add
 
 
 def edge_geom(pos, edge_index, edge_cell_shift, cell, batch, perm, lmax: int, n_basis: int = 0, r_start: float = 0.0,
@@ -611,7 +645,7 @@
     return agg
 
 
-def agg_linear(agg, species_order, wtab, io_table, blocks, d_out: int, add=None) -> torch.Tensor:
+def agg_linear(agg, species_order, wtab, io_table, blocks, d_out: int, add=None, add_species: bool = False) -> torch.Tensor:
     lib = _lib.load()
     from .plan import AGG_BLOCK, AGG_MAX_MT
     if lib.matten_agg_linear_block_chunks() != AGG_BLOCK or lib.matten_agg_linear_max_mt() != AGG_MAX_MT:
@@ -621,6 +655,16 @@
     n_rows, ld = agg.shape
     order, seg = species_order if species_order is not None else (None, None)
     n_species = wtab.shape[0] if wtab.dim() == 2 else 1
+    if add_species:
+        add = _species_add(add, n_species, d_out)
+        out = torch.empty(n_rows, d_out, dtype=torch.float32, device=agg.device)
+        with _timed(f"agg_linear/ld={ld}"):
+            rc = lib.matten_agg_linear_species_add(
+                _ptr(agg), ld, _ptr(order), _ptr(seg), n_species, _ptr(wtab), wtab.shape[-1], _ptr(io_table),
+                io_table.shape[0], _ptr(blocks), blocks.shape[0], _ptr(add), add.stride(0), d_out, n_rows, None, None,
+                None, None, 0, _ptr(out), _stream())
+        _lib.check(rc, "matten_agg_linear_species_add")
+        return out
     if add is not None:
         add = _need_rows(add, torch.float32, "add")
     out = torch.empty(n_rows, d_out, dtype=torch.float32, device=agg.device)
@@ -633,7 +677,7 @@
 
 
 def agg_linear_gate(agg, species_order, wtab, io_table, blocks, d_out: int, cmeta, act_cst, d_act: int, add=None,
-                    bn_scale=None, bn_shift=None) -> torch.Tensor:
+                    bn_scale=None, bn_shift=None, add_species: bool = False) -> torch.Tensor:
     lib = _lib.load()
     from .plan import AGG_BLOCK, AGG_GATE_SETS, AGG_MAX_MT
     if (lib.matten_agg_linear_block_chunks() != AGG_BLOCK or lib.matten_agg_linear_max_mt() != AGG_MAX_MT
@@ -644,7 +688,9 @@
     n_rows, ld = agg.shape
     order, seg = species_order if species_order is not None else (None, None)
     n_species = wtab.shape[0] if wtab.dim() == 2 else 1
-    if add is not None:
+    if add_species:
+        add = _species_add(add, n_species, d_out)
+    elif add is not None:
         add = _need_rows(add, torch.float32, "add")
     if cmeta.shape != (d_out, 4):
         raise ValueError("cmeta must be [d_out, 4]")
@@ -653,12 +699,12 @@
         if bn_scale.numel() != d_act or bn_shift.numel() != d_act:
             raise ValueError("bn_scale / bn_shift must have one value per activated column")
     out = torch.empty(n_rows, d_act, dtype=torch.float32, device=agg.device)
+    fn = lib.matten_agg_linear_species_add if add_species else lib.matten_agg_linear_gate
     with _timed(f"agg_linear/ld={ld}"):
-        rc = lib.matten_agg_linear_gate(_ptr(agg), ld, _ptr(order), _ptr(seg), n_species, _ptr(wtab), wtab.shape[-1],
-                                        _ptr(io_table), io_table.shape[0], _ptr(blocks), blocks.shape[0], _ptr(add),
-                                        add.stride(0) if add is not None else d_out, d_out, n_rows, _ptr(cmeta),
-                                        _ptr(act_cst), _ptr(bn_scale), _ptr(bn_shift), d_act, _ptr(out), _stream())
-    _lib.check(rc, "matten_agg_linear_gate")
+        rc = fn(_ptr(agg), ld, _ptr(order), _ptr(seg), n_species, _ptr(wtab), wtab.shape[-1], _ptr(io_table),
+                io_table.shape[0], _ptr(blocks), blocks.shape[0], _ptr(add), add.stride(0) if add is not None else d_out,
+                d_out, n_rows, _ptr(cmeta), _ptr(act_cst), _ptr(bn_scale), _ptr(bn_shift), d_act, _ptr(out), _stream())
+    _lib.check(rc, "matten_agg_linear_species_add" if add_species else "matten_agg_linear_gate")
     return out
 
 
```

Result: faster. 1.256 billion edge-TP/s, median of 6 (+1.2%).
